# dbdexter-dev/meteor_demod

Measured on AMD Instinct MI355X. Metric: IQ Msamples/s demodulated (whole node), higher is better.
Workload: dtype f32

## Files before the change

meteor_demod_amd/_capi.py:

```python
from __future__ import annotations

import ctypes as C
from pathlib import Path

import numpy as np

LIB_DIR = Path(__file__).resolve().parent / "lib"
LIB_PATH = LIB_DIR / "libmeteor_demod_amd.so"
import os as _os
if _os.environ.get("MDEMOD_LIB_PATH"):
    LIB_PATH = Path(_os.environ["MDEMOD_LIB_PATH"])

MDEMOD_OK = 0
MDEMOD_ERR_PARAM = -1
MDEMOD_ERR_NOMEM = -2
MDEMOD_ERR_HIP = -3
MDEMOD_ERR_OVERFLOW = -4
MDEMOD_ERR_RANGE = -5
MDEMOD_MAX_LOCK_EVENTS = 32
MDEMOD_FLAG_KERNEL_MASK, MDEMOD_FLAG_LAT_OFF, MDEMOD_FLAG_LAT_ON, MDEMOD_FLAG_V2_PACKED, MDEMOD_FLAG_NO_CLOCK_JUMP = 0x3, 0x4, 0x8, 0x10, 0x20


def variant_flags_from_env() -> int:
    f = {"v1": 1, "v3": 3}.get(_os.environ.get("MDEMOD_KERNEL", ""), 0)
# ... 27 lines not shown
        ("locked", C.c_int32), ("locked_once", C.c_int32), ("overflow", C.c_int32),
    ]


class MdemodLockEvent(C.Structure):
    _fields_ = [("symbol", C.c_uint64), ("locked", C.c_int32), ("pad", C.c_int32)]


class MdemodStreamState(C.Structure):
    _fields_ = [
        ("agc_gain", C.c_float), ("agc_bias_re", C.c_float), ("agc_bias_im", C.c_float),
        ("pll_phase", C.c_float), ("pll_freq", C.c_float), ("pll_err", C.c_float),
        ("pll_locked", C.c_int32), ("pll_locked_once", C.c_int32), ("pll_updown", C.c_int32),
        ("t_phase", C.c_float), ("t_freq", C.c_float), ("t_prev", C.c_float),
        ("t_dual_state", C.c_int32), ("oqpsk_inphase", C.c_float),
        ("n_samples", C.c_uint64), ("n_symbols", C.c_uint64),
        ("first_lock_symbol", C.c_int64),
    ]


class MdemodRecordingOpts(C.Structure):
    _fields_ = [("tile_samples", C.c_uint32), ("acquire_samples", C.c_uint32), ("frame_samples", C.c_uint32),
                ("settle_samples", C.c_uint32), ("pilot_block", C.c_uint32), ("pilot_margin_symbols", C.c_uint32),
                ("max_pilot_samples", C.c_uint64), ("match_symbols", C.c_uint32), ("repair", C.c_int32),
                ("carrier_seed", C.c_uint32), ("clock_seed", C.c_uint32), ("debug", C.c_int32), ("debug_tile", C.c_int32)]


class MdemodRecordingReport(C.Structure):
    _fields_ = [("n_symbols", C.c_uint64), ("pilot_samples", C.c_uint64), ("pilot_symbols", C.c_uint64),
                ("exact_symbols", C.c_uint64), ("first_lock_symbol", C.c_int64), ("samples_demodulated", C.c_uint64),
                ("n_tiles", C.c_uint32), ("tile_samples", C.c_uint32), ("weak_seams", C.c_uint32), ("seam_fixes", C.c_uint32),
                ("pilot_locked", C.c_int32), ("weak_carrier_tiles", C.c_uint32),
                ("pilot_seconds", C.c_double), ("tiles_seconds", C.c_double),
                ("frame_misses", C.c_uint32), ("repaired_tiles", C.c_uint32), ("rotation_jumps", C.c_uint32),
                ("frame_residual_rms", C.c_float), ("odd_tiles_kept", C.c_uint32), ("weak_clock_tiles", C.c_uint32)]


_P = C.POINTER
SIGNATURES = {
    "mdemod_abi_version": (C.c_uint32, []),
    "mdemod_last_error": (C.c_char_p, []),
    "mdemod_strerror": (C.c_char_p, [C.c_int]),
    "mdemod_init_device": (C.c_int, [C.c_int]),
    "mdemod_create": (C.c_int, [_P(MdemodParams), _P(C.c_void_p)]),
    "mdemod_destroy": (None, [C.c_void_p]),
    "mdemod_reset": (C.c_int, [C.c_void_p, C.c_void_p]),
    "mdemod_max_symbols": (C.c_uint64, [C.c_void_p, C.c_uint64]),
    "mdemod_process_device_uniform": (C.c_int, [C.c_void_p, C.c_void_p, C.c_uint64, C.c_uint32,
                                                C.c_void_p, C.c_uint64, C.c_uint32, C.c_void_p]),
    "mdemod_process_device": (C.c_int, [C.c_void_p, C.c_void_p, C.c_void_p, C.c_void_p,
                                        C.c_void_p, C.c_uint64, C.c_uint32, C.c_void_p]),
    "mdemod_process_host": (C.c_int, [C.c_void_p, _P(C.c_void_p), _P(C.c_uint32),
                                      _P(C.c_void_p), _P(C.c_uint32), _P(C.c_uint32)]),
    "mdemod_pin_host_buffer": (C.c_int, [C.c_void_p, C.c_void_p, C.c_size_t]),
    "mdemod_unpin_host_buffer": (C.c_int, [C.c_void_p, C.c_void_p]),
    "mdemod_get_status": (C.c_int, [C.c_void_p, C.c_uint32, C.c_uint32, _P(MdemodStatus), C.c_void_p]),
    "mdemod_get_lock_events": (C.c_int, [C.c_void_p, C.c_uint32, _P(MdemodLockEvent), C.c_uint32,
                                         _P(C.c_uint32), C.c_void_p]),
    "mdemod_get_state": (C.c_int, [C.c_void_p, C.c_uint32, _P(MdemodStreamState), C.c_void_p]),
    "mdemod_set_state": (C.c_int, [C.c_void_p, C.c_uint32, _P(MdemodStreamState), C.c_void_p]),
    "mdemod_set_state_all": (C.c_int, [C.c_void_p, _P(MdemodStreamState), C.c_void_p]),
    "mdemod_rotate_carrier": (C.c_int, [C.c_void_p, C.c_void_p, C.c_void_p]),
    "mdemod_set_carrier_seeds": (C.c_int, [C.c_void_p, C.c_void_p, C.c_void_p, C.c_void_p]),
    "mdemod_set_gain_seeds": (C.c_int, [C.c_void_p, C.c_void_p, C.c_void_p]),
    "mdemod_set_clock_seeds": (C.c_int, [C.c_void_p, C.c_void_p, C.c_void_p]),
    "mdemod_get_states": (C.c_int, [C.c_void_p, C.c_uint32, C.c_uint32, _P(MdemodStreamState), C.c_void_p]),
    "mdemod_copy_state": (C.c_int, [C.c_void_p, C.c_void_p, C.c_void_p]),
    "mdemod_nominal_pitch": (C.c_uint64, [C.c_void_p, C.c_uint64]),
    "mdemod_compact_soft": (C.c_int, [C.c_void_p, C.c_void_p, C.c_uint64, C.c_void_p, C.c_uint64, C.c_void_p]),
    "mdemod_fanin_peer": (C.c_int, [C.c_void_p, C.c_void_p, C.c_uint64, C.c_int, C.c_void_p, C.c_uint64, C.c_uint64, C.c_void_p, C.c_void_p]),
    "mdemod_carrier_window_samples": (C.c_uint32, [C.c_void_p, C.c_uint32]),
    "mdemod_estimate_carrier": (C.c_int, [C.c_void_p, C.c_void_p, C.c_uint64, C.c_void_p, C.c_uint32, C.c_uint32,
                                          C.c_void_p, C.c_void_p, C.c_void_p]),
    "mdemod_estimate_carrier_chirp": (C.c_int, [C.c_void_p, C.c_void_p, C.c_uint64, C.c_void_p, C.c_void_p, C.c_uint32, C.c_uint32,
                                                C.c_void_p, C.c_void_p, C.c_void_p]),
    "mdemod_estimate_clock": (C.c_int, [C.c_void_p, C.c_void_p, C.c_uint64, C.c_void_p, C.c_void_p, C.c_void_p, C.c_uint32, C.c_uint32,
                                        C.c_void_p, C.c_void_p, C.c_void_p]),
    "mdemod_kernel_name": (C.c_char_p, [C.c_void_p]),
    "mdemod_plan_kernel": (C.c_int, [C.c_void_p, C.c_char_p, C.c_uint32, C.POINTER(C.c_uint32), C.POINTER(C.c_uint32)]),
    "mdemod_clock_interp_magic": (C.c_uint32, [C.c_int32]),
    "mdemod_clock_table": (C.c_int, [C.c_int32, C.c_int32, _P(C.c_int32), C.c_uint32]),
    "mdemod_plan_clock_table": (C.c_int, [C.c_void_p, _P(C.c_int32), C.c_uint32]),
    "mdemod_plan_launch": (C.c_int, [C.c_void_p, _P(C.c_int32)]),
    "mdemod_device_count": (C.c_int, []),
    "mdemod_demodulate_recording_host": (C.c_int, [_P(MdemodParams), _P(MdemodRecordingOpts), C.c_void_p, C.c_uint64,
                                                   C.c_void_p, C.c_uint64, _P(MdemodRecordingReport)]),
    "mdemod_recording_default_opts": (None, [_P(MdemodRecordingOpts)]),
    "mdemod_demodulate_recording": (C.c_int, [_P(MdemodParams), _P(MdemodRecordingOpts), C.c_void_p, C.c_uint64,
                                              C.c_void_p, C.c_uint64, _P(MdemodRecordingReport), C.c_void_p]),
    "mdemod_history_len": (C.c_uint32, [C.c_void_p]),
    "mdemod_get_history": (C.c_int, [C.c_void_p, C.c_uint32, _P(C.c_float), C.c_void_p]),
    "mdemod_set_history": (C.c_int, [C.c_void_p, C.c_uint32, _P(C.c_float), C.c_void_p]),
    "mdemod_derive_tables": (C.c_int, [_P(MdemodParams), _P(C.c_float), C.c_uint32,
                                       _P(C.c_float), _P(C.c_float)]),
    "mdemod_get_rrc_table": (C.c_int, [C.c_void_p, _P(C.c_float), C.c_uint32]),
    "mdemod_get_loop_constants": (C.c_int, [C.c_void_p, _P(C.c_float)]),
    "mdemod_get_tanh_lut": (C.c_int, [C.c_void_p, _P(C.c_float)]),
    "mdemod_selftest_sincos": (C.c_int, [C.c_void_p, _P(C.c_float), C.c_uint32, _P(C.c_float), _P(C.c_float)]),
    "mdemod_selftest_hypot": (C.c_int, [C.c_void_p, _P(C.c_float), C.c_uint32, _P(C.c_float)]),
    "mdemod_selftest_turncode": (C.c_int, [C.c_void_p, _P(C.c_uint64), _P(C.c_uint64)]),
    "mdemod_selftest_sinlut": (C.c_int, [C.c_void_p, _P(C.c_uint64), _P(C.c_uint64)]),
    "mdemod_selftest_cabsf": (C.c_int, [C.c_void_p, C.c_uint64, _P(C.c_uint64), _P(C.c_uint64)]),
    "mdemod_selftest_seam_match": (C.c_int, [C.c_int, C.c_void_p, C.c_uint64, C.c_void_p, C.c_uint64, C.c_void_p, C.c_void_p, C.c_void_p,
                                             C.c_void_p, C.c_void_p, C.c_void_p, C.c_uint32, C.c_int, C.c_void_p, C.c_void_p, C.c_void_p, C.c_void_p]),
    "mdemod_selftest_assemble": (C.c_int, [C.c_void_p, C.c_uint64, C.c_void_p, C.c_uint64, C.c_void_p, C.c_void_p, C.c_void_p, C.c_void_p,
                                           C.c_void_p, C.c_void_p, C.c_uint32, C.c_void_p]),
    "mdemod_selftest_window_power": (C.c_int, [C.c_void_p, C.c_void_p, C.c_uint64, C.c_void_p, C.c_void_p, C.c_uint32, C.c_void_p, C.c_void_p]),
}

_lib = None


class MdemodError(RuntimeError):
    def __init__(self, code: int, what: str):
        self.code = code
        self.detail = last_error()
        super().__init__(f"{what}: error {code} ({strerror(code)})" + (f": {self.detail}" if self.detail else ""))


def hip_runtime_first() -> None:
    try:
        import torch
    except ImportError:
        pass


def lib() -> C.CDLL:
    global _lib
    if _lib is None:
        hip_runtime_first()
        if not LIB_PATH.exists():
            raise RuntimeError(
                f"{LIB_PATH} is missing: build the HIP extension first "
                "(python -m meteor_demod_amd.build). There is no CPU fallback.")
        _lib = _typed(C.CDLL(str(LIB_PATH)), SIGNATURES, missing_ok=bool(_os.environ.get("MDEMOD_LIB_PATH")))
    return _lib


def _typed(handle: C.CDLL, *tables: dict, missing_ok: bool = False) -> C.CDLL:
    for table in tables:
        for name, (res, args) in table.items():
            if missing_ok and not hasattr(handle, name):
                continue
            fn = getattr(handle, name)
            fn.restype = res
            fn.argtypes = args
    return handle


def bind(*tables: dict) -> C.CDLL:
    return _typed(lib(), *tables)


def take_bytes(ptr, count: int, dtype=np.uint8) -> np.ndarray:
    dtype = np.dtype(dtype)
    return np.frombuffer(C.string_at(ptr, count * dtype.itemsize), dtype=dtype).copy() if count else np.zeros(0, dtype=dtype)


def strerror(code: int) -> str:
    return lib().mdemod_strerror(code).decode()


def last_error() -> str:
    fn = getattr(lib(), "mdemod_last_error", None)
    return (fn() or b"").decode(errors="replace") if fn is not None else ""

# ... 6 lines not shown
```

meteor_demod_amd/csrc/demod_api.cpp:

```cpp
#include <hip/hip_runtime.h>

#include <cmath>
#include <cstdio>
#include <cstdlib>
#include <cstring>
#include <new>
#include <vector>

#include "demod_host.h"
#include "demod_internal.h"
#include "hip_host.h"

struct mdemod_ctx {
	mdemod_params params;
	HostTables    tab;
	int           block_threads;
	size_t        lds_bytes;
	size_t        sample_bytes;

	DemodStateSoA st;
	float        *d_ctab;
	float        *d_lut;
	int32_t      *d_clock_tab;
	float        *d_rrc;
	int           hyb_block;
	bool          v1_global_table;
	bool          use_rot;
	bool          lat_ok;
	int           lat_ring, lat_span;
	size_t        lat_lds;
	MdmDevMem     mem;

	void   *pipe;
};

namespace {

template <typename T>
int
fetch(const T *dev, uint32_t first, uint32_t count, std::vector<T> &host, hipStream_t st)
{
	host.resize(count);
	HIP_TRY(hipMemcpyAsync(host.data(), dev + first, sizeof(T) * count, hipMemcpyDeviceToHost, st));
	return MDEMOD_OK;
}

bool
wants_latency_kernel(const mdemod_ctx *ctx)
{
	if (!ctx->lat_ok || (ctx->params.reserved & MDEMOD_FLAG_LAT_OFF)) return false;
	if (ctx->params.reserved & MDEMOD_FLAG_LAT_ON) return true;
	const double per_firing = static_cast<double>(ctx->tab.osf) / (ctx->params.oqpsk ? 2.0 : 1.0);
	if (ctx->tab.use_rw && per_firing > 32.0) return false;
	const uint32_t most = (ctx->tab.use_rw && (ctx->tab.rw_mid || ctx->tab.rw_far)) ? 1024u : (per_firing >= 8.0 ? 2048u : 4096u);
	return ctx->params.n_streams <= most;
}

struct LaunchPick {
	int kind;
	int geom;
	int many_slides;
	int compact;
	int long_filter;
};

LaunchPick
pick_launch(const mdemod_ctx *ctx)
{
	LaunchPick p = { MDEMOD_LAUNCH_V1, 0, 0, 0, 0 };
	const int geom = ctx->tab.rw_mid ? 1 : (ctx->tab.rw_far ? 2 : 0);
	if (wants_latency_kernel(ctx)) p.kind = MDEMOD_LAUNCH_LAT;
	else if (ctx->tab.use_rw && ctx->tab.rw_gather) { p.kind = MDEMOD_LAUNCH_GAT; p.long_filter = ctx->tab.c.taps > 65 ? 1 : 0; }
	else if (ctx->tab.use_rw && ctx->tab.rw_hyb) {
		p.kind = MDEMOD_LAUNCH_ROTH; p.geom = geom;
		p.many_slides = static_cast<double>(ctx->tab.osf) / (ctx->params.oqpsk ? 2.0 : 1.0) > 20.0 ? 1 : 0;
	}
	else if (ctx->tab.use_rw && ctx->use_rot) { p.kind = MDEMOD_LAUNCH_ROT; p.compact = ctx->tab.rw_std_compact ? 1 : 0; }
	else if (ctx->tab.use_rw && ctx->tab.rw_compact4) { p.kind = MDEMOD_LAUNCH_ROTP; p.geom = geom; }
	else if (ctx->tab.use_rw) p.kind = -1;
	return p;
}

int
launch(mdemod_ctx *ctx, DemodLaunch &L, hipStream_t stream)
{
	L.c = ctx->tab.c;
	L.st = ctx->st;
	L.n_streams = ctx->params.n_streams;
	L.ctab = ctx->d_ctab;
	L.ctab_floats = static_cast<uint32_t>(ctx->tab.ctab.size());
	L.tanh_lut = ctx->d_lut;
	L.c.clock_tab = ctx->d_clock_tab;
	const LaunchPick p = pick_launch(ctx);
	switch (p.kind) {
// ... 597 lines not shown
mdemod_fanin_peer(mdemod_ctx *src, const int8_t *soft_dev, uint64_t soft_stride_symbols, int dst_device,
                  int8_t *dst_soft_dev, uint64_t pitch_symbols, uint64_t first_row, uint32_t *dst_counts_dev, void *hip_stream)
try { MDEMOD_API_ENTER
	if (!src || !soft_dev || !dst_soft_dev || (soft_stride_symbols & 7) || (pitch_symbols & 7) || dst_device < 0) return MDEMOD_ERR_PARAM;
	int rc = mdm_select_device(src->params.device);
	if (rc) return rc;
	const int src_device = src->params.device;
	if (dst_device != src_device) {
		int can = 0;
		HIP_TRY(hipDeviceCanAccessPeer(&can, src_device, dst_device));
		if (!can) {
			mdm_note_error("mdemod_fanin_peer: device %d cannot reach the memory of device %d (no peer access between them)", src_device, dst_device);
			return MDEMOD_ERR_HIP;
		}
		const hipError_t e = hipDeviceEnablePeerAccess(dst_device, 0);
		if (e == hipErrorPeerAccessAlreadyEnabled) (void)hipGetLastError();
		else HIP_TRY(e);
	}
	hipStream_t st = static_cast<hipStream_t>(hip_stream);
	const uint32_t n = src->params.n_streams;
	HIP_TRY(mdemod_launch_compact_rows(soft_dev, soft_stride_symbols, dst_soft_dev + 2 * first_row * pitch_symbols, pitch_symbols,
	                                   src->st.sym_this_call, n, st));
	if (dst_counts_dev)
		HIP_TRY(hipMemcpyPeerAsync(dst_counts_dev + first_row, dst_device, src->st.sym_this_call, src_device, sizeof(uint32_t) * n, st));
	return MDEMOD_OK;
} MDEMOD_API_CATCH

const char *
mdemod_kernel_name(const mdemod_ctx *ctx)
{
	if (!ctx) return "";
	if (wants_latency_kernel(ctx)) return "demod_kernel_lat (one stream per wave: FIR farm + serial scalar stage)";
	if (!ctx->tab.use_rw) return "demod_kernel (v1 LDS ring)";
	if (ctx->tab.rw_gather) return ctx->tab.c.taps > 65 ? "demod_kernel_gat (v3 gather: sample rates beyond every window, 129 taps, every firing loads its own taps)"
	                                                     : "demod_kernel_gat (v3 gather: sample rates beyond every window, 65 taps, every firing loads its own taps)";
	if (ctx->tab.rw_hyb && ctx->tab.rw_far) return "demod_kernel_roth (v3 hybrid window, far: float input, 65 taps at up to 54 samples per firing, 80 slots in VGPRs + 40 in AccVGPRs)";
	if (ctx->tab.rw_hyb) return ctx->tab.rw_mid ? "demod_kernel_roth (v3 hybrid window, mid: float input, 65 taps at up to 30 samples per firing, 80 slots in VGPRs + 16 in AccVGPRs)"
	                                            : "demod_kernel_roth (v3 hybrid window: float input, 129 taps, 80 slots in VGPRs + 80 in AccVGPRs)";
	if (ctx->tab.rw_compact4) return ctx->tab.rw_wide ? "demod_kernel_rotp (v3 rotating packed window, wide: 129 taps at up to 30 samples per firing)"
	                                 : (ctx->tab.rw_mid ? "demod_kernel_rotp (v3 rotating packed window, mid: 65 taps at up to 15 samples per firing)"
	                                                    : "demod_kernel_rotp (v3 rotating packed window, far: 65 taps at up to 46 samples per firing)");
	return "demod_kernel_rot (v3 rotating register window)";
}

int
mdemod_plan_kernel(const mdemod_params *params, char *name, uint32_t name_cap, uint32_t *lds_bytes, uint32_t *block_threads)
try { MDEMOD_API_ENTER
	if (!params || !name || name_cap == 0 || params->n_streams == 0) return MDEMOD_ERR_PARAM;
	mdemod_ctx *ctx = new (std::nothrow) mdemod_ctx();
	if (!ctx) return MDEMOD_ERR_NOMEM;
	ctx->params = *params;
	ctx->pipe = nullptr;
	const int rc = plan_context(ctx);
	if (rc == MDEMOD_OK) {
		snprintf(name, name_cap, "%s%s", mdemod_kernel_name(ctx), ctx->v1_global_table && !wants_latency_kernel(ctx) ? " [table in global memory]" : "");
		if (lds_bytes) *lds_bytes = static_cast<uint32_t>(wants_latency_kernel(ctx) ? ctx->lat_lds : ctx->lds_bytes);
		if (block_threads) *block_threads = wants_latency_kernel(ctx) ? 64u : static_cast<uint32_t>(ctx->tab.use_rw ? (ctx->tab.rw_wide ? MDEMOD_RW_WIDE_BLOCK : (ctx->tab.c.sin_lut ? MDEMOD_RW_LUT_BLOCK : MDEMOD_RW_BLOCK)) : ctx->block_threads);
	}
	delete ctx;
	return rc;
} MDEMOD_API_CATCH

int
mdemod_plan_clock_table(const mdemod_params *params, int32_t *out, uint32_t cap_entries)
try { MDEMOD_API_ENTER
	if (!params || params->n_streams == 0) return MDEMOD_ERR_PARAM;
	mdemod_ctx *ctx = new (std::nothrow) mdemod_ctx();
	if (!ctx) return MDEMOD_ERR_NOMEM;
	ctx->params = *params;
	ctx->pipe = nullptr;
	int rc = plan_context(ctx);
	if (rc == MDEMOD_OK) {
		const size_t entries = ctx->tab.clock_tab.size() / 4;
		if (out && entries > cap_entries) rc = MDEMOD_ERR_PARAM;
		else {
			if (out && entries) memcpy(out, ctx->tab.clock_tab.data(), ctx->tab.clock_tab.size() * sizeof(int32_t));
			rc = static_cast<int>(entries);
		}
	}
	delete ctx;
	return rc;
} MDEMOD_API_CATCH

int
mdemod_plan_launch(const mdemod_params *params, int32_t out[MDEMOD_PLAN_LAUNCH_WORDS])
try { MDEMOD_API_ENTER
	if (!params || !out || params->n_streams == 0) return MDEMOD_ERR_PARAM;
	mdemod_ctx *ctx = new (std::nothrow) mdemod_ctx();
	if (!ctx) return MDEMOD_ERR_NOMEM;
	ctx->params = *params;
	ctx->pipe = nullptr;
	int rc = plan_context(ctx);
	if (rc == MDEMOD_OK) {
		const LaunchPick p = pick_launch(ctx);
		const DemodConsts &c = ctx->tab.c;
		const bool lat = p.kind == MDEMOD_LAUNCH_LAT, v1 = p.kind == MDEMOD_LAUNCH_V1;
		const int32_t v[MDEMOD_PLAN_LAUNCH_WORDS] = {
			p.kind, params->bps, c.oqpsk ? 1 : 0, c.step_safe, c.sin_lut ? 1 : 0, ctx->tab.clock_tab.empty() ? 0 : 1,
			p.geom, p.many_slides, p.compact, p.long_filter,
			v1 ? ctx->block_threads : 0, v1 && ctx->v1_global_table ? 1 : 0, v1 ? c.win_granules : 0,
			lat && ctx->tab.use_rw ? 1 : 0, 0, 0 };
		memcpy(out, v, sizeof(v));
		if (p.kind < 0) rc = MDEMOD_ERR_PARAM;
	}
	delete ctx;
	return rc;
} MDEMOD_API_CATCH

uint32_t
mdemod_history_len(const mdemod_ctx *ctx)
{
	return ctx ? static_cast<uint32_t>(ctx->tab.c.hpad) : 0;
}

int
mdemod_get_history(mdemod_ctx *ctx, uint32_t stream, float *iq_pairs, void *hip_stream)
try { MDEMOD_API_ENTER
	if (!ctx || !iq_pairs) return MDEMOD_ERR_PARAM;
	if (stream >= ctx->params.n_streams) return MDEMOD_ERR_RANGE;
	int rc = mdm_select_device(ctx->params.device);
	if (rc) return rc;
	hipStream_t st = static_cast<hipStream_t>(hip_stream);
	const int hfmt = ctx->tab.use_rw ? 32 : ctx->params.bps;
	const size_t sb = 2 * static_cast<size_t>(hfmt) / 8, ns = ctx->params.n_streams;
	const int hpad = ctx->tab.c.hpad;
	std::vector<unsigned char> raw(static_cast<size_t>(hpad) * sb);
	if (ctx->tab.use_rw)
		HIP_TRY(hipMemcpyAsync(raw.data(), static_cast<const unsigned char *>(ctx->st.hist) + static_cast<size_t>(stream) * hpad * sb,
		                       static_cast<size_t>(hpad) * sb, hipMemcpyDeviceToHost, st));
	else
		HIP_TRY(hipMemcpy2DAsync(raw.data(), sb, static_cast<const unsigned char *>(ctx->st.hist) + stream * sb,
		                         ns * sb, sb, hpad, hipMemcpyDeviceToHost, st));
	HIP_TRY(hipStreamSynchronize(st));
	for (int k = 0; k < hpad; k++) {
		const unsigned char *p = &raw[k * sb];
		if (hfmt == 8) { iq_pairs[2*k] = (float)((int)p[0] - 128); iq_pairs[2*k+1] = (float)((int)p[1] - 128); }
		else if (hfmt == 16) { int16_t v[2]; memcpy(v, p, 4); iq_pairs[2*k] = v[0]; iq_pairs[2*k+1] = v[1]; }
		else memcpy(&iq_pairs[2*k], p, 8);
	}
	return MDEMOD_OK;
} MDEMOD_API_CATCH

int
mdemod_set_history(mdemod_ctx *ctx, uint32_t stream, const float *iq_pairs, void *hip_stream)
try { MDEMOD_API_ENTER
	if (!ctx || !iq_pairs) return MDEMOD_ERR_PARAM;
	if (stream >= ctx->params.n_streams) return MDEMOD_ERR_RANGE;
	int rc = mdm_select_device(ctx->params.device);
	if (rc) return rc;
	hipStream_t st = static_cast<hipStream_t>(hip_stream);
	const int hfmt = ctx->tab.use_rw ? 32 : ctx->params.bps;
	const size_t sb = 2 * static_cast<size_t>(hfmt) / 8, ns = ctx->params.n_streams;
	const int hpad = ctx->tab.c.hpad;
	std::vector<unsigned char> raw(static_cast<size_t>(hpad) * sb);
	for (int k = 0; k < hpad; k++) {
		unsigned char *p = &raw[k * sb];
		const float re = iq_pairs[2*k], im = iq_pairs[2*k+1];
		if (hfmt == 8) {
			if (re != floorf(re) || im != floorf(im) || re < -128 || re > 127 || im < -128 || im > 127) return MDEMOD_ERR_PARAM;
			p[0] = (unsigned char)((int)re + 128); p[1] = (unsigned char)((int)im + 128);
		} else if (hfmt == 16) {
			if (re != floorf(re) || im != floorf(im) || re < -32768 || re > 32767 || im < -32768 || im > 32767) return MDEMOD_ERR_PARAM;
			int16_t v[2] = { (int16_t)re, (int16_t)im }; memcpy(p, v, 4);
		} else memcpy(p, &iq_pairs[2*k], 8);
	}
	if (ctx->tab.use_rw)
// ... 107 lines not shown
```

meteor_demod_amd/csrc/demod_kernel_gat.hip:

```cpp
#include "rotwin_body.h"
#include "hip_host.h"

namespace {

typedef float gpair_t __attribute__((ext_vector_type(2)));
typedef float gquad_t __attribute__((ext_vector_type(4)));
typedef __attribute__((address_space(3))) const gquad_t lds_gquad;
typedef __attribute__((address_space(3))) const float lds_gfloat;

template <int FMT> struct GFmt;
template <> struct GFmt<16> {
	enum { G = 4 };
	__device__ static __forceinline__ gpair_t get(const uint4 &q, int k) { const uint32_t w = (&q.x)[k]; return gpair_t{ (float)(int)(int16_t)(w & 0xFFFFu), (float)((int)w >> 16) }; }
	__device__ static __forceinline__ gpair_t one(uint32_t w) { return gpair_t{ (float)(int)(int16_t)(w & 0xFFFFu), (float)((int)w >> 16) }; }
};
template <> struct GFmt<8> {
	enum { G = 8 };
	__device__ static __forceinline__ gpair_t get(const uint4 &q, int k) { const uint32_t w = (&q.x)[k >> 1] >> (16 * (k & 1)); return gpair_t{ (float)((int)(w & 0xFFu) - 128), (float)((int)((w >> 8) & 0xFFu) - 128) }; }
	__device__ static __forceinline__ gpair_t one(uint16_t w) { return gpair_t{ (float)((int)(w & 0xFFu) - 128), (float)((int)(w >> 8) - 128) }; }
};
template <> struct GFmt<32> {
	enum { G = 2 };
	__device__ static __forceinline__ gpair_t get(const uint4 &q, int k) { return gpair_t{ __uint_as_float((&q.x)[2 * k]), __uint_as_float((&q.x)[2 * k + 1]) }; }
	__device__ static __forceinline__ gpair_t one(float2 w) { return gpair_t{ w.x, w.y }; }
};

template <int KT, int FMT>
struct WinG {
	static constexpr int G = GFmt<FMT>::G, kTaps = KT, kBack = KT - 1, AMAX = G - 1, NS = KT + AMAX, NW = 4 * ((NS + 3) / 4), SLIDE = 4, MAXSL = 1, DEPTH = 1,
	                     BLOCK = MDEMOD_RW_BLOCK, ROTN = 1, RING = 32, REGSLOTS = 0;
	static constexpr bool GATHER = true, SCALAR_SLIDE = false, VCONST = false;
	static_assert(NS % G == 0 && NS / G <= 36, "whole 16-byte loads, and few enough of them to stay in registers");
	typedef typename RFmt<FMT>::sample_t sample_t;
	__device__ __forceinline__ void setup(uint32_t) {}
	__device__ static __forceinline__ void put_history(const float2 *, bool, int) {}
	__device__ static __forceinline__ void put_init(const RGran<FMT> (&)[1], int) {}
	__device__ static __forceinline__ void put(const RGran<FMT> (&)[1], int) {}
	__device__ static __forceinline__ void fir(uint32_t, int, int, const DemodConsts &, int, float &, float &) {}

	__device__ static __forceinline__ void
	fir_gather(uint32_t ctab_addr, const sample_t *src, const float2 *hist, int v, int n, int bank, const DemodConsts &C, float &re, float &im)
	{
		const int oldest = v - kBack - (KT - 1);
		const int d = oldest & (G - 1);
		const int start = oldest - d;
		const int o = AMAX - d;
		const uint32_t row = ctab_addr + 4u * (uint32_t)(__mul24(bank * 4 + (o & 3), C.ctab_row_stride) + (o & ~3));
		gpair_t acc = { 0.0f, 0.0f };
		if (__builtin_expect(md_all(start >= 0 && start + NS <= n), 1)) {
			uint4 raw[NS / G];
#pragma unroll
			for (int g = 0; g < NS / G; g++) __builtin_memcpy(&raw[g], src + start + G * g, 16);
#pragma unroll
			for (int s4 = 0; s4 < NS / 4; s4++) {
				gquad_t c = { 0.0f, 0.0f, 0.0f, 0.0f };
				c = *(lds_gquad *)(row + 16u * (uint32_t)s4);
				const float cf[4] = { c.x, c.y, c.z, c.w };
#pragma unroll
				for (int k = 0; k < 4; k++) {
					const int slot = 4 * s4 + k;
					const gpair_t smp = GFmt<FMT>::get(raw[slot / G], slot % G);
					const gpair_t p = smp * cf[k];
					acc = acc + p;
				}
			}
			if constexpr (NS % 4 != 0) {
#pragma unroll
				for (int slot = NS / 4 * 4; slot < NS; slot++) {
					const float cf = *(lds_gfloat *)(row + 4u * (uint32_t)slot);
					const gpair_t p = GFmt<FMT>::get(raw[slot / G], slot % G) * cf;
					acc = acc + p;
				}
			}
		} else {
#pragma unroll 1
			for (int k = 0; k < KT; k++) {
				const int idx = oldest + k;
				gpair_t smp;
				if (idx < 0) { const float2 h = hist[kBack + idx]; smp.x = h.x; smp.y = h.y; }
				else smp = GFmt<FMT>::one(src[idx]);
				const float cf = *(lds_gfloat *)(row + 4u * (uint32_t)(d + k));
				const gpair_t p = smp * cf;
				acc = acc + p;
			}
		}
		re = acc.x; im = acc.y;
	}
};

template <int FMT, int OQPSK, int KT>
__global__ void __launch_bounds__(MDEMOD_RW_BLOCK, 2)
demod_kernel_gat(const DemodLaunch L)
{
	rotwin_demod<WinG<KT, FMT>, FMT, OQPSK, 0>(L);
}

template <int FMT, int OQPSK, int KT>
hipError_t
launch_gat(const DemodLaunch &L, size_t lds_bytes, hipStream_t stream)
{
	const uint32_t blocks = (L.n_streams + MDEMOD_RW_BLOCK - 1) / MDEMOD_RW_BLOCK;
	auto kfn = demod_kernel_gat<FMT, OQPSK, KT>;
	return mdm_launch(kfn, dim3(blocks), dim3(MDEMOD_RW_BLOCK), lds_bytes, stream, L);
}

}

template <int FMT>
static hipError_t
launch_gat_fmt(const DemodLaunch &L, int long_filter, size_t lds_bytes, hipStream_t stream)
{
	if constexpr (FMT != 32)
		if (long_filter) return L.c.oqpsk ? launch_gat<FMT, 1, 129>(L, lds_bytes, stream) : launch_gat<FMT, 0, 129>(L, lds_bytes, stream);
// ... 15 lines not shown
```

meteor_demod_amd/csrc/demod_kernel_rot.hip:

```cpp
#include "rotwin_body.h"
#include "rot_fir_bounds.h"
#include "hip_host.h"
#ifdef ROTWIN_ASM_HEADER
#include ROTWIN_ASM_HEADER
#else
#include "rotwin_asm.h"
#endif

namespace {

static_assert(ROTWIN_NCH * 8 == 80 && ROTWIN_SLIDE == 8, "window = ten chunks of eight, a slide brings one");


__device__ __forceinline__ void
rot_fir(uint32_t row_addr, int rot, int flags, float &re, float &im)
{
	int tmp;
#if ROTWIN_PK == 1 || ROTWIN_PK == 3
	typedef float pair_t __attribute__((ext_vector_type(2)));
	pair_t acc, p0, p1;
	asm volatile(ROTWIN_FIR_ASM
	             : [acc] "=&v"(acc), [p0] "=&v"(p0), [p1] "=&v"(p1), [tmp] "=&s"(tmp)
	             : [addr] "v"(row_addr), [rot] "s"(rot), [flags] "s"(flags)
	             : "vcc", "scc", ROTWIN_COEF_CLOBBERS);
	re = acc.x; im = acc.y;
#else
	float t0, t1, t2, t3;
	asm volatile(ROTWIN_FIR_ASM
	             : [ar] "=&v"(re), [ai] "=&v"(im), [t0] "=&v"(t0), [t1] "=&v"(t1), [t2] "=&v"(t2), [t3] "=&v"(t3), [tmp] "=&s"(tmp)
	             : [addr] "v"(row_addr), [rot] "s"(rot), [flags] "s"(flags)
	             : "vcc", "scc", ROTWIN_COEF_CLOBBERS);
#endif
}

template <int FMT> __device__ __forceinline__ void rot_put(const RGran<FMT> &a, const RGran<FMT> &b, int &q, int &base);
template <> __device__ __forceinline__ void
rot_put<16>(const RGran<16> &a, const RGran<16> &b, int &q, int &base)
{
	int tmp;
	asm volatile(ROTWIN_PUT_S16_ASM
	             : [tmp] "=&s"(tmp), [rot] "+s"(q), [base] "+s"(base)
	             : [g0] "v"(a.w[0]), [g1] "v"(a.w[1]), [g2] "v"(a.w[2]), [g3] "v"(a.w[3]),
	               [g4] "v"(b.w[0]), [g5] "v"(b.w[1]), [g6] "v"(b.w[2]), [g7] "v"(b.w[3])
	             : "vcc", "scc", "v255", "memory");
}
template <> __device__ __forceinline__ void
rot_put<8>(const RGran<8> &a, const RGran<8> &b, int &q, int &base)
{
	const uint32_t g0 = a.w[0] ^ 0x80808080u, g1 = a.w[1] ^ 0x80808080u, g2 = b.w[0] ^ 0x80808080u, g3 = b.w[1] ^ 0x80808080u;
	int tmp;
	asm volatile(ROTWIN_PUT_U8_ASM
	             : [tmp] "=&s"(tmp), [rot] "+s"(q), [base] "+s"(base)
	             : [g0] "v"(g0), [g1] "v"(g1), [g2] "v"(g2), [g3] "v"(g3)
	             : "vcc", "scc", "v255", "memory");
}
__device__ __forceinline__ void
rot_put_floats(const uint32_t (&f)[16], int &q, int &base)
{
	int tmp;
	asm volatile(ROTWIN_PUT_F32_ASM
	             : [tmp] "=&s"(tmp), [rot] "+s"(q), [base] "+s"(base)
	             : [f0] "v"(f[0]), [f1] "v"(f[1]), [f2] "v"(f[2]), [f3] "v"(f[3]), [f4] "v"(f[4]), [f5] "v"(f[5]), [f6] "v"(f[6]), [f7] "v"(f[7]),
	               [f8] "v"(f[8]), [f9] "v"(f[9]), [f10] "v"(f[10]), [f11] "v"(f[11]), [f12] "v"(f[12]), [f13] "v"(f[13]), [f14] "v"(f[14]), [f15] "v"(f[15])
	             : "vcc", "scc", "v255", "memory");
}
__device__ __forceinline__ void
rot_put_floats(const uint32_t (&f)[16], int q)
{
	int base = 0;
	rot_put_floats(f, q, base);
}
template <> __device__ __forceinline__ void
rot_put<32>(const RGran<32> &a, const RGran<32> &b, int &q, int &base)
{
	uint32_t f[16];
#pragma unroll
	for (int i = 0; i < 8; i++) { f[i] = a.w[i]; f[8 + i] = b.w[i]; }
	rot_put_floats(f, q, base);
}

template <int FMT, int COMPACT = 0, int BLK = MDEMOD_RW_BLOCK, int VC = 0, int RSL = 0>
struct WinF {
	static constexpr int kTaps = 65, kBack = 64, NW = 80, SLIDE = 8, AMAX = NW - kTaps, MAXSL = 1, DEPTH = 1, BLOCK = BLK, ROTN = NW / SLIDE, RING = 32;
	static constexpr bool GATHER = false;
	static constexpr bool SCALAR_SLIDE = true;
	static constexpr bool VCONST = VC != 0;
	static_assert(SLIDE == ROTWIN_SLIDE && ROTN == ROTWIN_NCH, "the slide's assembly counts for itself");
	__device__ __forceinline__ void setup(uint32_t) {}
	static constexpr int REGSLOTS = RSL;
	__device__ static __forceinline__ void put_history(const float2 *hist, bool valid, int q)
	{
		const uint4 *h4 = reinterpret_cast<const uint4 *>(hist);
		uint32_t f[16];
#pragma unroll
		for (int i = 0; i < 4; i++) {
			uint4 h = h4[i];
			if (!valid) h = make_uint4(0, 0, 0, 0);
			f[4 * i] = h.x; f[4 * i + 1] = h.y; f[4 * i + 2] = h.z; f[4 * i + 3] = h.w;
		}
		rot_put_floats(f, q);
	}
	__device__ static __forceinline__ void put(const RGran<FMT> (&g)[2], int q) { int base = 0; rot_put<FMT>(g[0], g[1], q, base); }
	__device__ static __forceinline__ void put_init(const RGran<FMT> (&g)[2], int q) { put(g, q); }
	__device__ static __forceinline__ void slide(const RGran<FMT> (&g)[2], int &rot, int &base) { rot_put<FMT>(g[0], g[1], rot, base); }
	__device__ static __forceinline__ void fir(uint32_t ctab_addr, int a, int bank, const DemodConsts &C, int rot, float &re, float &im)
	{
		const int o = AMAX - a;
		uint32_t row_addr;
		if (COMPACT) row_addr = rot_mad24((uint32_t)(bank * 4 + (o & 3)), 4u * (uint32_t)C.ctab_row_stride, ctab_addr + 4u * (uint32_t)(o & ~3));
		else row_addr = rot_mad24(rot_mad24((uint32_t)a, (uint32_t)C.interp, (uint32_t)bank), 4u * (uint32_t)C.ctab_row_stride, ctab_addr);
		static_assert(AMAX == 15, "two bits of a / 4");
		const uint64_t ex = __builtin_amdgcn_ballot_w64(true);
		const RotFirQ q = rot_fir_q(ex, __builtin_amdgcn_ballot_w64(a >= 4), __builtin_amdgcn_ballot_w64(a >= 8), __builtin_amdgcn_ballot_w64(a >= 12));
		int q_hi = q.q_hi;
		asm("" : "+s"(q_hi));
		const int flags = rot_fir_flags(q.q_lo, q_hi);
#ifdef ROT_EXP_NOSKIP
		int f0 = __builtin_amdgcn_readfirstlane(flags);
		asm volatile("s_and_b32 %0, %0, 0" : "+s"(f0) : : "scc");
		rot_fir(row_addr, rot, f0, re, im);
#else
		rot_fir(row_addr, rot, flags, re, im);
#endif
	}
};

typedef float pair_t2 __attribute__((ext_vector_type(2)));

template <int NA>
__device__ __forceinline__ void
rot_fir_acc(uint32_t addr, int rot, int last, pair_t2 &acc)
{
	int tmp;
	if constexpr (NA == 10)
		asm volatile(ROTWIN_FIR_ACC_ASM
		             : [acc] "+v"(acc), [tmp] "=&s"(tmp)
		             : [addr] "v"(addr), [rot] "s"(rot), [last] "s"(last)
		             : "vcc", "scc", ROTWIN_COEF_CLOBBERS, ROTWIN_ACC_CLOBBERS);
	else if constexpr (NA == 2)
		asm volatile(ROTWIN_FIR_ACC2_ASM
		             : [acc] "+v"(acc), [tmp] "=&s"(tmp)
		             : [addr] "v"(addr), [rot] "s"(rot), [last] "s"(last)
		             : "vcc", "scc", ROTWIN_COEF_CLOBBERS, ROTWIN_ACC_CLOBBERS);
	else
		asm volatile(ROTWIN_FIR_ACC5_ASM
		             : [acc] "+v"(acc), [tmp] "=&s"(tmp)
		             : [addr] "v"(addr), [rot] "s"(rot), [last] "s"(last)
		             : "vcc", "scc", ROTWIN_COEF_CLOBBERS, ROTWIN_ACC_CLOBBERS);
}
#define ROT_F16_OPERANDS \
	[f0] "v"(f[0]), [f1] "v"(f[1]), [f2] "v"(f[2]), [f3] "v"(f[3]), [f4] "v"(f[4]), [f5] "v"(f[5]), [f6] "v"(f[6]), [f7] "v"(f[7]), \
	[f8] "v"(f[8]), [f9] "v"(f[9]), [f10] "v"(f[10]), [f11] "v"(f[11]), [f12] "v"(f[12]), [f13] "v"(f[13]), [f14] "v"(f[14]), [f15] "v"(f[15])
template <int NA>
__device__ __forceinline__ void
rot_migrate(const uint32_t (&f)[16], int q)
{
	int tmp;
	if constexpr (NA == 10)
		asm volatile(ROTWIN_MIGRATE_ASM : [tmp] "=&s"(tmp) : ROT_F16_OPERANDS, [rot] "s"(q) : "vcc", "scc", "v255", ROTWIN_ACC_CLOBBERS, "memory");
	else if constexpr (NA == 2)
		asm volatile(ROTWIN_MIGRATE2_ASM : [tmp] "=&s"(tmp) : ROT_F16_OPERANDS, [rot] "s"(q) : "vcc", "scc", "v255", ROTWIN_ACC_CLOBBERS, "memory");
	else
		asm volatile(ROTWIN_MIGRATE5_ASM : [tmp] "=&s"(tmp) : ROT_F16_OPERANDS, [rot] "s"(q) : "vcc", "scc", "v255", ROTWIN_ACC_CLOBBERS, "memory");
}
template <int NA>
__device__ __forceinline__ void
rot_put_acc(const uint32_t (&f)[16], int q)
{
	int tmp;
	if constexpr (NA == 10)
		asm volatile(ROTWIN_PUT_ACC_ASM : [tmp] "=&s"(tmp) : ROT_F16_OPERANDS, [rot] "s"(q) : "vcc", "scc", ROTWIN_ACC_CLOBBERS, "memory");
	else if constexpr (NA == 2)
		asm volatile(ROTWIN_PUT_ACC2_ASM : [tmp] "=&s"(tmp) : ROT_F16_OPERANDS, [rot] "s"(q) : "vcc", "scc", ROTWIN_ACC_CLOBBERS, "memory");
	else
		asm volatile(ROTWIN_PUT_ACC5_ASM : [tmp] "=&s"(tmp) : ROT_F16_OPERANDS, [rot] "s"(q) : "vcc", "scc", ROTWIN_ACC_CLOBBERS, "memory");
}

template <int BLK, int NA, int MSL>
struct WinH {
	static constexpr int NR = 10, SLIDE = 8, NW = SLIDE * (NR + NA), kTaps = NA == 10 ? 129 : 65, kBack = kTaps - 1, AMAX = NW - kTaps, MAXSL = MSL, DEPTH = MSL,
	                     BLOCK = BLK, ROTN = NR, RING = 32, REGSLOTS = 0;
	static constexpr bool GATHER = false, SCALAR_SLIDE = false, VCONST = false;
	static_assert((NA == 10 || NA == 2 || NA == 5) && AMAX == (NA == 5 ? 55 : 31) && kBack % SLIDE == 0, "wide (160 slots, 129 taps), mid (96 slots, 65 taps) or far (120 slots, 65 taps)");
	__device__ __forceinline__ void setup(uint32_t) {}
	__device__ static __forceinline__ void place(const uint32_t (&f)[16], int c)
	{
		if (c < NR) rot_put_floats(f, c);
		else rot_put_acc<NA>(f, c - NR);
	}
	__device__ static __forceinline__ void put_history(const float2 *hist, bool valid, int c)
	{
		const uint4 *h4 = reinterpret_cast<const uint4 *>(hist);
		uint32_t f[16];
#pragma unroll
		for (int i = 0; i < 4; i++) {
			uint4 h = h4[i];
			if (!valid) h = make_uint4(0, 0, 0, 0);
			f[4 * i] = h.x; f[4 * i + 1] = h.y; f[4 * i + 2] = h.z; f[4 * i + 3] = h.w;
		}
		place(f, c);
	}
	__device__ static __forceinline__ void put_init(const RGran<32> (&g)[2], int c)
	{
		uint32_t f[16];
#pragma unroll
		for (int i = 0; i < 8; i++) { f[i] = g[0].w[i]; f[8 + i] = g[1].w[i]; }
		place(f, c);
	}
	__device__ static __forceinline__ void put(const RGran<32> (&g)[2], int q)
	{
		uint32_t f[16];
#pragma unroll
		for (int i = 0; i < 8; i++) { f[i] = g[0].w[i]; f[8 + i] = g[1].w[i]; }
		rot_migrate<NA>(f, q);
	}
	__device__ static __forceinline__ void fir(uint32_t ctab_addr, int a, int bank, const DemodConsts &C, int rot, float &re, float &im)
	{
		const int o = AMAX - a;
		const uint32_t row = ctab_addr + 4u * (uint32_t)(__mul24(bank * 4 + (o & 3), C.ctab_row_stride) + (o & ~3));
		const int flags = (md_all(a >= 8) ? 3 : 0) | ((NA != 10 && md_all(a <= 7)) ? 16 : 0);
		rot_fir(row, rot, __builtin_amdgcn_readfirstlane(flags), re, im);
		if (NA == 10 || md_any(a >= 16)) {
			int last;
			if (NA == 10) last = 6 + (md_any(a >= 8) ? 1 : 0) + (md_any(a >= 16) ? 1 : 0) + (md_any(a >= 24) ? 1 : 0);
			else {
				last = md_any(a >= 24) ? 1 : 0;
				if (NA == 5) last += (md_any(a >= 32) ? 1 : 0) + (md_any(a >= 40) ? 1 : 0) + (md_any(a >= 48) ? 1 : 0);
			}
			pair_t2 acc = { re, im };
			rot_fir_acc<NA>(row + 4u * 80u, NA == 10 ? rot : (NA == 2 ? (rot & 1) : (rot >= 5 ? rot - 5 : rot)), __builtin_amdgcn_readfirstlane(last), acc);
			re = acc.x; im = acc.y;
		}
	}
};

template <int OQPSK, int BLK, int NA, int MSL>
__global__ void __launch_bounds__(BLK, 1) __attribute__((amdgpu_num_vgpr(ROTWIN_LIMIT)))
demod_kernel_roth(const DemodLaunch L)
{
	rotwin_demod<WinH<BLK, NA, MSL>, 32, OQPSK, 0>(L);
}

#ifndef ROT_VCONST
#define ROT_VCONST 1
#endif
template <int FMT, int OQPSK, int KS, int COMPACT, int LUT>
constexpr int rot_regslots() { return 15; }
template <int FMT, int OQPSK, int KS, int COMPACT, int LUT>
__global__ void __launch_bounds__(LUT ? MDEMOD_RW_LUT_BLOCK : MDEMOD_RW_BLOCK, 2) __attribute__((amdgpu_num_vgpr(ROTWIN_LIMIT / 2)))
demod_kernel_rot(const DemodLaunch L)
{
	rotwin_demod<WinF<FMT, COMPACT, LUT ? MDEMOD_RW_LUT_BLOCK : MDEMOD_RW_BLOCK, ROT_VCONST, rot_regslots<FMT, OQPSK, KS, COMPACT, LUT>()>, FMT, OQPSK, KS, LUT>(L);
}

template <int FMT, int OQPSK, int KS, int COMPACT = 0, int LUT = 0>
hipError_t
launch_rot_ks(const DemodLaunch &L, size_t lds_bytes, hipStream_t stream)
{
	constexpr int BLOCK = LUT ? MDEMOD_RW_LUT_BLOCK : MDEMOD_RW_BLOCK;
	const uint32_t blocks = (L.n_streams + BLOCK - 1) / BLOCK;
	auto kfn = demod_kernel_rot<FMT, OQPSK, KS, COMPACT, LUT>;
	return mdm_launch(kfn, dim3(blocks), dim3(BLOCK), lds_bytes, stream, L);
}

template <int FMT, int OQPSK>
hipError_t
launch_rot(const DemodLaunch &L, int compact, size_t lds_bytes, hipStream_t stream)
{
	constexpr int KS = OQPSK ? 6 : 14;
	if (compact) return launch_rot_ks<FMT, OQPSK, 0, 1>(L, lds_bytes, stream);
	return L.c.sin_lut && L.c.step_safe == KS && L.c.clock_tab ? launch_rot_ks<FMT, OQPSK, KS, 0, 1>(L, lds_bytes, stream) : launch_rot_ks<FMT, OQPSK, 0>(L, lds_bytes, stream);
}

}

template <int OQPSK, int BLK, int NA, int MSL>
static hipError_t
launch_roth(const DemodLaunch &L, size_t lds_bytes, hipStream_t stream)
{
	const uint32_t blocks = (L.n_streams + BLK - 1) / BLK;
	auto kfn = demod_kernel_roth<OQPSK, BLK, NA, MSL>;
	return mdm_launch(kfn, dim3(blocks), dim3(BLK), lds_bytes, stream, L);
}

hipError_t
mdemod_launch_demod_roth(const DemodLaunch &L, int geom, int many_slides, size_t lds_bytes, hipStream_t stream)
{
	if (geom == 1 && many_slides) return L.c.oqpsk ? launch_roth<1, 256, 2, 3>(L, lds_bytes, stream) : launch_roth<0, 256, 2, 3>(L, lds_bytes, stream);
	if (geom == 1) return L.c.oqpsk ? launch_roth<1, 256, 2, 2>(L, lds_bytes, stream) : launch_roth<0, 256, 2, 2>(L, lds_bytes, stream);
	if (geom == 2) return L.c.oqpsk ? launch_roth<1, 256, 5, 3>(L, lds_bytes, stream) : launch_roth<0, 256, 5, 3>(L, lds_bytes, stream);
	return L.c.oqpsk ? launch_roth<1, 256, 10, 2>(L, lds_bytes, stream) : launch_roth<0, 256, 10, 2>(L, lds_bytes, stream);
}

hipError_t
mdemod_launch_demod_rot(const DemodLaunch &L, int fmt, int compact, size_t lds_bytes, hipStream_t stream)
{
	switch (fmt) {
	case 16: return L.c.oqpsk ? launch_rot<16, 1>(L, compact, lds_bytes, stream) : launch_rot<16, 0>(L, compact, lds_bytes, stream);
	case 8:  return L.c.oqpsk ? launch_rot<8, 1>(L, compact, lds_bytes, stream) : launch_rot<8, 0>(L, compact, lds_bytes, stream);
	case 32: return L.c.oqpsk ? launch_rot<32, 1>(L, compact, lds_bytes, stream) : launch_rot<32, 0>(L, compact, lds_bytes, stream);
	default: return hipErrorInvalidValue;
	}
}
```

meteor_demod_amd/csrc/demod_kernel_rotp.hip:

```cpp
#include "rotwin_body.h"
#include "hip_host.h"
#ifdef ROTPK_ASM_HEADER
#include ROTPK_ASM_HEADER
#else
#include "rotpk_asm.h"
#endif

namespace {

typedef float pair_t __attribute__((ext_vector_type(2)));

template <int GEO> struct GeoP;
#ifndef ROTP_WIDE_DEPTH
#define ROTP_WIDE_DEPTH 1
#endif
#ifndef ROTP_MID_DEPTH
#define ROTP_MID_DEPTH 1
#endif
#ifndef ROTP_FAR_DEPTH
#define ROTP_FAR_DEPTH 2
#endif
template <> struct GeoP<0> { static constexpr int kTaps = 129, NW = MDEMOD_RW_WIDE_NW, MAXSL = 1, DEPTH = ROTP_WIDE_DEPTH, BLOCK = MDEMOD_RW_WIDE_BLOCK; };
template <> struct GeoP<1> { static constexpr int kTaps = 65, NW = MDEMOD_RW_MID_NW, MAXSL = 1, DEPTH = ROTP_MID_DEPTH, BLOCK = MDEMOD_RW_BLOCK; };
#ifndef ROTP_FAR_MAXSL
#define ROTP_FAR_MAXSL 2
#endif
template <> struct GeoP<2> { static constexpr int kTaps = 65, NW = MDEMOD_RW_FAR_NW, MAXSL = ROTP_FAR_MAXSL, DEPTH = ROTP_FAR_DEPTH, BLOCK = MDEMOD_RW_BLOCK; };
static_assert(MDEMOD_RW_WIDE_NW == 160 && MDEMOD_RW_MID_NW == 96 && MDEMOD_RW_FAR_NW == 112, "gen_rotpk_asm.py: GEOS");

template <int GEO, int FMT> struct AsmP;
#if ROTPK_FORM == 0
#define ROTP_FIR_CALL(TEXT, CLOB)                                                                                             \
	float ar = 0.0f, ai = 0.0f;                                                                                               \
	asm volatile(TEXT : [ar] "+v"(ar), [ai] "+v"(ai), [addr] "+v"(addr), [cnt] "+s"(cnt), [tmp] "=&s"(tmp)                    \
	             : [entry] "s"(entry), [sub] "s"(sub) : "vcc", "scc", CLOB);                                                \
	re = ar; im = ai;
#else
#define ROTP_FIR_CALL(TEXT, CLOB)                                                                                             \
	pair_t acc = { 0.0f, 0.0f };                                                                                              \
	asm volatile(TEXT : [acc] "+v"(acc), [addr] "+v"(addr), [cnt] "+s"(cnt), [tmp] "=&s"(tmp)                                 \
	             : [entry] "s"(entry), [sub] "s"(sub) : "vcc", "scc", CLOB);                                                \
	re = acc.x; im = acc.y;
#endif
#define ROTP_ASM(GEO, NAME, FMT)                                                                                              \
	template <> struct AsmP<GEO, FMT> {                                                                                       \
		__device__ static __forceinline__ void fir(uint32_t addr, int entry, int sub, int cnt, float &re, float &im)          \
		{                                                                                                                     \
			int tmp;                                                                                                          \
			ROTP_FIR_CALL(ROTPK_##NAME##_##FMT##_FIR_ASM, ROTPK_##NAME##_##FMT##_CLOBBERS)                                     \
		}                                                                                                                     \
		__device__ static __forceinline__ void put(const uint32_t (&g)[FMT == 16 ? 16 : 8], int q);                           \
	};
ROTP_ASM(0, WIDE, 16) ROTP_ASM(0, WIDE, 8) ROTP_ASM(1, MID, 16) ROTP_ASM(1, MID, 8) ROTP_ASM(2, FAR, 16) ROTP_ASM(2, FAR, 8)

#define ROTP_PUT16(GEO, NAME)                                                                                                 \
	__device__ __forceinline__ void AsmP<GEO, 16>::put(const uint32_t (&g)[16], int q)                                        \
	{                                                                                                                         \
		int tmp;                                                                                                              \
		asm volatile(ROTPK_##NAME##_16_PUT_ASM                                                                                \
		             : [tmp] "=&s"(tmp)                                                                                       \
		             : [g0] "v"(g[0]), [g1] "v"(g[1]), [g2] "v"(g[2]), [g3] "v"(g[3]), [g4] "v"(g[4]), [g5] "v"(g[5]), [g6] "v"(g[6]),  \
		               [g7] "v"(g[7]), [g8] "v"(g[8]), [g9] "v"(g[9]), [g10] "v"(g[10]), [g11] "v"(g[11]), [g12] "v"(g[12]),  \
		               [g13] "v"(g[13]), [g14] "v"(g[14]), [g15] "v"(g[15]), [rot] "s"(q)                                     \
		             : "vcc", "scc", "v255", "memory");                                                                       \
	}
#define ROTP_PUT8(GEO, NAME)                                                                                                  \
	__device__ __forceinline__ void AsmP<GEO, 8>::put(const uint32_t (&g)[8], int q)                                          \
	{                                                                                                                         \
		int tmp;                                                                                                              \
		asm volatile(ROTPK_##NAME##_8_PUT_ASM                                                                                 \
		             : [tmp] "=&s"(tmp)                                                                                       \
		             : [g0] "v"(g[0]), [g1] "v"(g[1]), [g2] "v"(g[2]), [g3] "v"(g[3]), [g4] "v"(g[4]), [g5] "v"(g[5]), [g6] "v"(g[6]),  \
		               [g7] "v"(g[7]), [rot] "s"(q)                                                                           \
		             : "vcc", "scc", "v255", "memory");                                                                       \
	}
ROTP_PUT16(0, WIDE) ROTP_PUT16(1, MID) ROTP_PUT16(2, FAR) ROTP_PUT8(0, WIDE) ROTP_PUT8(1, MID) ROTP_PUT8(2, FAR)

template <int GEO, int FMT>
struct WinP {
	static constexpr int kTaps = GeoP<GEO>::kTaps, kBack = kTaps - 1, NW = GeoP<GEO>::NW, SLIDE = 16, AMAX = NW - kTaps,
	                     MAXSL = GeoP<GEO>::MAXSL, DEPTH = GeoP<GEO>::DEPTH, BLOCK = GeoP<GEO>::BLOCK, NCH = NW / SLIDE, GD = FMT == 16 ? 16 : 8, REGSLOTS = 0, ROTN = NCH, RING = 32;
	static constexpr bool GATHER = false, SCALAR_SLIDE = false, VCONST = false;
	__device__ __forceinline__ void setup(uint32_t) {}
	static_assert(kBack % SLIDE == 0 && NW % SLIDE == 0, "history and window are whole chunks");

	__device__ static __forceinline__ void put_history(const float2 *hist, bool valid, int q)
	{
		uint32_t g[GD];
#pragma unroll
		for (int k = 0; k < 16; k++) {
			float2 h = hist[k];
			if (!valid) h = make_float2(0.0f, 0.0f);
			if (FMT == 16) {
				g[k] = ((uint32_t)(int)h.x & 0xFFFFu) | ((uint32_t)(int)h.y << 16);
			} else {
				const uint32_t s = (uint32_t)(((int)h.x + 128) & 0xFF) | ((uint32_t)(((int)h.y + 128) & 0xFF) << 8);
				if (k & 1) g[k / 2] |= s << 16; else g[k / 2] = s;
			}
		}
		AsmP<GEO, FMT>::put(g, q);
	}
	__device__ static __forceinline__ void put(const RGran<FMT> (&gr)[4], int q)
	{
		uint32_t g[GD];
#pragma unroll
		for (int i = 0; i < 4; i++)
#pragma unroll
			for (int j = 0; j < GD / 4; j++) g[i * (GD / 4) + j] = gr[i].w[j];
		AsmP<GEO, FMT>::put(g, q);
	}
	__device__ static __forceinline__ void put_init(const RGran<FMT> (&gr)[4], int q) { put(gr, q); }
	__device__ static __forceinline__ void fir(uint32_t ctab_addr, int a, int bank, const DemodConsts &C, int rot, float &re, float &im)
	{
		const int o = AMAX - a;
		uint32_t addr = rot_mad24((uint32_t)(bank * 4 + (o & 3)), 4u * (uint32_t)C.ctab_row_stride, ctab_addr + 4u * (uint32_t)(o & ~3));
		constexpr int QB = AMAX / 4 >= 8 ? 4 : 3;
		static_assert(AMAX / 4 < (1 << QB) && (kTaps - 1) % 4 == 0, "alignments in groups of four");
		int q_lo = 0, q_hi = (1 << QB) - 1;
#pragma unroll
		for (int b = QB - 1; b >= 0; b--) {
			const int t = q_lo + (1 << b);
			q_lo = md_all(a >= 4 * t) ? t : q_lo;
			const int u = q_hi - (1 << b);
			q_hi = md_all(a < 4 * (u + 1)) ? u : q_hi;
		}
		q_lo = __builtin_amdgcn_readfirstlane(q_lo); q_hi = __builtin_amdgcn_readfirstlane(q_hi);
		const int c_lo = q_lo >> 2;
		int chunk = rot + c_lo;
		chunk = chunk >= NCH ? chunk - NCH : chunk;
		const int sub = q_lo & 3;
		constexpr int XS = ROTPK_EXIT / 4;
		const int cnt = (q_hi + (kTaps - 1) / 4) / XS - q_lo / XS;
		AsmP<GEO, FMT>::fir(addr + 64u * (uint32_t)c_lo, __builtin_amdgcn_readfirstlane(chunk), __builtin_amdgcn_readfirstlane(sub), __builtin_amdgcn_readfirstlane(cnt), re, im);
	}
};

#define ROTP_KERNEL(GEO, NAME, FMT, OQ)                                                                                       \
	__global__ void __launch_bounds__(GeoP<GEO>::BLOCK, 2) __attribute__((amdgpu_num_vgpr(ROTPK_##NAME##_##FMT##_LIMIT / 2)))  \
	demod_kernel_rotp_##NAME##_##FMT##_##OQ(const DemodLaunch L) { rotwin_demod<WinP<GEO, FMT>, FMT, OQ, 0>(L); }
__global__ void __launch_bounds__(GeoP<0>::BLOCK, 2) __attribute__((amdgpu_num_vgpr(ROTPK_WIDE_16_LIMIT / 2)))
demod_kernel_rotp_WIDE_16_0_ks109(const DemodLaunch L) { rotwin_demod<WinP<0, 16>, 16, 0, 109, 1>(L); }
ROTP_KERNEL(0, WIDE, 16, 0) ROTP_KERNEL(0, WIDE, 16, 1) ROTP_KERNEL(0, WIDE, 8, 0) ROTP_KERNEL(0, WIDE, 8, 1)
ROTP_KERNEL(1, MID, 16, 0) ROTP_KERNEL(1, MID, 16, 1) ROTP_KERNEL(1, MID, 8, 0) ROTP_KERNEL(1, MID, 8, 1)
ROTP_KERNEL(2, FAR, 16, 0) ROTP_KERNEL(2, FAR, 16, 1) ROTP_KERNEL(2, FAR, 8, 0) ROTP_KERNEL(2, FAR, 8, 1)

typedef void (*rotp_kernel_t)(const DemodLaunch);

hipError_t
launch_rotp(rotp_kernel_t kfn, int block, const DemodLaunch &L, size_t lds_bytes, hipStream_t stream)
{
	const uint32_t blocks = (L.n_streams + block - 1) / block;
	return mdm_launch(kfn, dim3(blocks), dim3(block), lds_bytes, stream, L);
}

}

hipError_t
mdemod_launch_demod_rotp(const DemodLaunch &L, int fmt, int geom , size_t lds_bytes, hipStream_t stream)
{
	if ((fmt != 16 && fmt != 8) || geom < 0 || geom > 2) return hipErrorInvalidValue;
	static const rotp_kernel_t table[3][2][2] = {
		{ { demod_kernel_rotp_WIDE_16_0, demod_kernel_rotp_WIDE_16_1 }, { demod_kernel_rotp_WIDE_8_0, demod_kernel_rotp_WIDE_8_1 } },
		{ { demod_kernel_rotp_MID_16_0, demod_kernel_rotp_MID_16_1 }, { demod_kernel_rotp_MID_8_0, demod_kernel_rotp_MID_8_1 } },
		{ { demod_kernel_rotp_FAR_16_0, demod_kernel_rotp_FAR_16_1 }, { demod_kernel_rotp_FAR_8_0, demod_kernel_rotp_FAR_8_1 } },
// ... 6 lines not shown
```

meteor_demod_amd/csrc/gen_rotwin_asm.py:

```python
#!/usr/bin/env python3
import os
import sys

WB = 96
CB = None
NCH = 10
SLIDE = 8
PAIRWAIT = int(os.environ.get("ROTWIN_PAIRWAIT", "1"))
DC = int(os.environ.get("ROTWIN_DC", "1"))
NBUF = 2 * (DC + 1) if PAIRWAIT else 4
CB = 96 - 4 * NBUF
PK = int(os.environ.get("ROTWIN_PK", "1"))
TB = CB - 4
CHB = 32


def q(lines):
    return "\n".join('\t"%s\\n\\t"' % l for l in lines)


def jump(tag, n):
    return [
        "s_getpc_b64 vcc",
        ".L%s_pc_%%=:" % tag,
# ... 14 lines not shown
    if PK in (0, 2):
        L += ["v_mov_b32 %[ar], 0", "v_mov_b32 %[ai], 0"]
    else:
        L += ["v_mov_b64 %[acc], 0"]
    L += [load(h) for h in range(2 * DC if PAIRWAIT else D)]
    L += jump("fir", NCH)
    for r in range(NCH):
        L += [".Lfir_%d_%%=:" % r]
        for h in range(NH):
            c = h // 2
            if PAIRWAIT:
                if h % 2 == 0:
                    L += [load(x) for x in (h + 2 * DC, h + 2 * DC + 1) if x < NH]
                    L += ["s_waitcnt lgkmcnt(%d)" % min(2 * DC, max(0, NH - 2 - h))]
            else:
                if h + D < NH:
                    L += [load(h + D)]
                L += ["s_waitcnt lgkmcnt(%d)" % min(D, NH - 1 - h)]
            if h < 3:
                L += ["s_bitcmp1_b32 %%[flags], %d" % h, "s_cbranch_scc1 .Lfir_%d_s%d_%%=" % (r, h)]
            if h >= NH - 3:
                L += ["s_bitcmp1_b32 %%[flags], %d" % (3 + NH - 1 - h), "s_cbranch_scc1 .Lfir_%d_s9_%%=" % r]
            hb = CB + 4 * (h % NBUF)
            wq = WB + 16 * ((c + r) % NCH) + 8 * (h & 1)
            if PK == 1:
                def mul(j):
                    return ["v_pk_mul_f32 %%[p%d], v[%d:%d], v[%d:%d] op_sel:[0,%d] op_sel_hi:[1,%d]"
                            % (j & 1, wq + 2 * j, wq + 2 * j + 1, hb + 2 * (j // 2), hb + 2 * (j // 2) + 1, j & 1, j & 1)]
                def add(j):
                    return ["v_pk_add_f32 %%[acc], %%[acc], %%[p%d]" % (j & 1)]
            elif PK == 2:
                def mul(j):
                    t = TB + 2 * (j & 1)
                    return ["v_pk_mul_f32 v[%d:%d], v[%d:%d], v[%d:%d] op_sel:[0,%d] op_sel_hi:[1,%d]"
                            % (t, t + 1, wq + 2 * j, wq + 2 * j + 1, hb + 2 * (j // 2), hb + 2 * (j // 2) + 1, j & 1, j & 1)]
                def add(j):
                    t = TB + 2 * (j & 1)
                    return ["v_add_f32 %%[ar], %%[ar], v%d" % t, "v_add_f32 %%[ai], %%[ai], v%d" % (t + 1)]
            elif PK == 3:
                def mul(j):
                    t = TB + 2 * (j & 1)
                    return ["v_mul_f32 v%d, v%d, v%d" % (t, hb + j, wq + 2 * j), "v_mul_f32 v%d, v%d, v%d" % (t + 1, hb + j, wq + 2 * j + 1)]
                def add(j):
                    t = TB + 2 * (j & 1)
                    return ["v_pk_add_f32 %%[acc], %%[acc], v[%d:%d]" % (t, t + 1)]
            else:
                def mul(j):
                    t = "%%[t%d]" % (2 * (j & 1)), "%%[t%d]" % (2 * (j & 1) + 1)
                    return ["v_mul_f32 %s, v%d, v%d" % (t[0], hb + j, wq + 2 * j),
                            "v_mul_f32 %s, v%d, v%d" % (t[1], hb + j, wq + 2 * j + 1)]
                def add(j):
                    t = "%%[t%d]" % (2 * (j & 1)), "%%[t%d]" % (2 * (j & 1) + 1)
                    return ["v_add_f32 %%[ar], %%[ar], %s" % t[0], "v_add_f32 %%[ai], %%[ai], %s" % t[1]]
            L += mul(0)
            for j in range(4):
                if j + 1 < 4:
                    L += mul(j + 1)
                L += add(j)
            if h < 3:
                L += [".Lfir_%d_s%d_%%=:" % (r, h)]
        L += [".Lfir_%d_s9_%%=:" % r, "s_branch .Lfir_end_%="]
    L += [".Lfir_end_%=:", "s_waitcnt lgkmcnt(0)"]
    return L


def put(kind):
    L = ["s_nop 1"] if kind == "u8" else []
    L += jump("put", NCH)
    for r in range(NCH):
        L += [".Lput_%d_%%=:" % r]
        wq = WB + 16 * r
        for s in range(8):
            for comp in range(2):
                dst = wq + 2 * s + comp
                if kind == "s16":
                    L += ["v_cvt_f32_i32_sdwa v%d, sext(%%[g%d]) dst_sel:DWORD dst_unused:UNUSED_PAD src0_sel:WORD_%d" % (dst, s, comp)]
                elif kind == "u8":
                    L += ["v_cvt_f32_i32_sdwa v%d, sext(%%[g%d]) dst_sel:DWORD dst_unused:UNUSED_PAD src0_sel:BYTE_%d" % (dst, s // 2, 2 * (s & 1) + comp)]
                else:
                    L += ["v_mov_b32 v%d, %%[f%d]" % (dst, 2 * s + comp)]
        L += ["s_branch .Lput_end_%="]
    L += [".Lput_end_%=:"]
    L += ["s_add_i32 %%[base], %%[base], %d" % SLIDE,
          "s_add_i32 %[rot], %[rot], 1",
          "s_cmp_eq_u32 %%[rot], %d" % NCH,
          "s_cselect_b32 %[rot], 0, %[rot]"]
    return L


AB = 96


def fir_acc(NA, tag):
    NH = 2 * NA
    lo = 6 if NA == NCH else 0
    def load(h):
        b = CB + 4 * (h % 3)
        return "ds_read_b128 v[%d:%d], %%[addr] offset:%d" % (b, b + 3, 16 * h)
    L = [load(h) for h in range(2)]
    L += jump(tag, NA)
    for r in range(NA):
        L += [".L%s_%d_%%=:" % (tag, r)]
        for h in range(NH):
            c = h // 2
            if h + 2 < NH:
                L += [load(h + 2)]
            L += ["s_waitcnt lgkmcnt(%d)" % min(2, NH - 1 - h)]
            hb = CB + 4 * (h % 3)
            aq = AB + 16 * ((c + r) % NA) + 8 * (h & 1)
            def rd(j):
                t = CB + 12 + 2 * (j & 1)
                return ["v_accvgpr_read_b32 v%d, a%d" % (t, aq + 2 * j), "v_accvgpr_read_b32 v%d, a%d" % (t + 1, aq + 2 * j + 1)]
            def mul(j):
                t = CB + 12 + 2 * (j & 1)
                return ["v_pk_mul_f32 v[%d:%d], v[%d:%d], v[%d:%d] op_sel:[0,%d] op_sel_hi:[1,%d]" % (t, t + 1, t, t + 1, hb + 2 * (j // 2), hb + 2 * (j // 2) + 1, j & 1, j & 1)]
            def add(j):
                t = CB + 12 + 2 * (j & 1)
                return ["v_pk_add_f32 %%[acc], %%[acc], v[%d:%d]" % (t, t + 1)]
            L += rd(0) + rd(1) + mul(0) + mul(1) + add(0) + rd(2) + add(1) + rd(3) + mul(2) + mul(3) + add(2) + add(3)
            if h % 2 == 1 and lo <= c < NA - 1:
                L += ["s_cmp_eq_u32 %%[last], %d" % c, "s_cbranch_scc1 .L%s_end_%%=" % tag]
        L += ["s_branch .L%s_end_%%=" % tag]
    L += [".L%s_end_%%=:" % tag, "s_waitcnt lgkmcnt(0)"]
    return L


def migrate(NA, tag):
    assert NCH % NA == 0
    L = jump(tag, NCH)
    for r in range(NCH):
        L += [".L%s_%d_%%=:" % (tag, r)]
        L += ["v_accvgpr_read_b32 v%d, a%d" % (WB + 16 * r + k, AB + 16 * (r % NA) + k) for k in range(16)]
        L += ["v_accvgpr_write_b32 a%d, %%[f%d]" % (AB + 16 * (r % NA) + k, k) for k in range(16)]
        L += ["s_branch .L%s_end_%%=" % tag]
    L += [".L%s_end_%%=:" % tag]
    return L


def put_acc(NA, tag):
    L = jump(tag, NA)
    for r in range(NA):
        L += [".L%s_%d_%%=:" % (tag, r)]
        L += ["v_accvgpr_write_b32 a%d, %%[f%d]" % (AB + 16 * r + k, k) for k in range(16)]
        L += ["s_branch .L%s_end_%%=" % tag]
    L += [".L%s_end_%%=:" % tag]
    return L


def main():
    out = []
    out.append("/* GENERATED by gen_rotwin_asm.py - do not edit.  gfx950 assembly of the rotating register window. */")
    out.append("#ifndef MDEMOD_ROTWIN_ASM_H")
    out.append("#define MDEMOD_ROTWIN_ASM_H")
    out.append("#define ROTWIN_WB %d" % WB)
    out.append("#define ROTWIN_CB %d" % CB)
    out.append("#define ROTWIN_LIMIT %d   /* first register the compiler may not use */" % (TB if PK in (2, 3) else CB))
    out.append("#define ROTWIN_NCH %d" % NCH)
    out.append("#define ROTWIN_SLIDE %d" % SLIDE)
    out.append("#define ROTWIN_AB %d   /* first AccVGPR of the hybrid window's newer half */" % AB)
    out.append("#define ROTWIN_PK %d" % PK)
    out.append("#define ROTWIN_FIR_ASM \\\n" + q(fir()).replace("\n", " \\\n"))
    for kind in ("s16", "u8", "f32"):
        out.append("#define ROTWIN_PUT_%s_ASM \\\n" % kind.upper() + q(put(kind)).replace("\n", " \\\n"))
    for NA, sfx in ((NCH, ""), (2, "2"), (5, "5")):
        out.append("#define ROTWIN_FIR_ACC%s_ASM \\\n" % sfx + q(fir_acc(NA, "fira" + sfx)).replace("\n", " \\\n"))
        out.append("#define ROTWIN_MIGRATE%s_ASM \\\n" % sfx + q(migrate(NA, "mig" + sfx)).replace("\n", " \\\n"))
# ... 10 lines not shown
```

meteor_demod_amd/csrc/mdemod_internal_api.h:

```cpp
#ifndef MDEMOD_INTERNAL_API_H
#define MDEMOD_INTERNAL_API_H

#include "../../include/meteor_demod_amd.h"

#ifdef __cplusplus
#include <new>
void mdm_note_error(const char *fmt, ...) __attribute__((format(printf, 1, 2)));
struct mdm_api_scope { mdm_api_scope(); ~mdm_api_scope(); };
#define MDEMOD_API_ENTER mdm_api_scope api_scope_;
#define MDEMOD_API_CATCH catch (...) { mdm_note_error("a C++ exception reached the boundary (allocation failed, or a thread could not be started)"); return MDEMOD_ERR_NOMEM; }
extern "C" {
#endif


int  mdemod_set_state_all(mdemod_ctx *ctx, const mdemod_stream_state *seed, void *hip_stream);
int  mdemod_rotate_carrier(mdemod_ctx *ctx, const int32_t *quarter_turns_dev, void *hip_stream);

int  mdemod_set_carrier_seeds(mdemod_ctx *ctx, const float *freq_dev, const int32_t *updown_dev, void *hip_stream);
int  mdemod_set_gain_seeds(mdemod_ctx *ctx, const float *gain_dev, void *hip_stream);

int  mdemod_set_clock_seeds(mdemod_ctx *ctx, const float *t_freq_dev, void *hip_stream);
int  mdemod_get_states(mdemod_ctx *ctx, uint32_t first, uint32_t count, mdemod_stream_state *out, void *hip_stream);
int  mdemod_copy_state(mdemod_ctx *dst, mdemod_ctx *src, void *hip_stream);

uint32_t mdemod_carrier_window_samples(const mdemod_params *params, uint32_t window_samples);
int  mdemod_estimate_carrier(const mdemod_params *params, const void *iq_dev, uint64_t n_samples,
                             const uint64_t *starts_dev, uint32_t n_windows, uint32_t window_samples,
                             float *freq_dev, float *quality_dev, void *hip_stream);
int  mdemod_estimate_carrier_chirp(const mdemod_params *params, const void *iq_dev, uint64_t n_samples,
                                   const uint64_t *starts_dev, const float *chirp_dev, uint32_t n_windows, uint32_t window_samples,
                                   float *freq_dev, float *quality_dev, void *hip_stream);
int  mdemod_estimate_clock(const mdemod_params *params, const void *iq_dev, uint64_t n_samples,
                           const uint64_t *starts_dev, const float *carrier_dev, const float *chirp_dev,
                           uint32_t n_windows, uint32_t window_samples, float *t_freq_dev, float *quality_dev, void *hip_stream);


int  mdemod_derive_tables(const mdemod_params *params, float *rrc_out, uint32_t rrc_cap,
                          float consts_out[8], float lut_out[32]);
int  mdemod_plan_kernel(const mdemod_params *params, char *name, uint32_t name_cap, uint32_t *lds_bytes, uint32_t *block_threads);

uint32_t mdemod_clock_interp_magic(int32_t interp);
int  mdemod_clock_table(int32_t interp, int32_t k_safe, int32_t *out, uint32_t cap_entries);
int  mdemod_plan_clock_table(const mdemod_params *params, int32_t *out, uint32_t cap_entries);

enum { MDEMOD_LAUNCH_LAT = 0, MDEMOD_LAUNCH_GAT = 1, MDEMOD_LAUNCH_ROTH = 2, MDEMOD_LAUNCH_ROT = 3, MDEMOD_LAUNCH_ROTP = 4, MDEMOD_LAUNCH_V1 = 5 };
#define MDEMOD_PLAN_LAUNCH_WORDS 16
int  mdemod_plan_launch(const mdemod_params *params, int32_t out[MDEMOD_PLAN_LAUNCH_WORDS]);

int  mdemod_get_rrc_table(const mdemod_ctx *ctx, float *out, uint32_t cap);
int  mdemod_get_loop_constants(const mdemod_ctx *ctx, float out[8]);
int  mdemod_get_tanh_lut(const mdemod_ctx *ctx, float out[32]);

int  mdemod_selftest_sincos(mdemod_ctx *ctx, const float *x, uint32_t n,
                            float *sin_out, float *cos_out);
int  mdemod_selftest_hypot(mdemod_ctx *ctx, const float *xy, uint32_t n_pairs, float *out);
int  mdemod_selftest_turncode(mdemod_ctx *ctx, uint64_t *n_checked, uint64_t *n_mismatch);
int  mdemod_selftest_cabsf(mdemod_ctx *ctx, uint64_t pairs, uint64_t *n_mismatch, uint64_t *n_fallback);
int  mdemod_selftest_sinlut(mdemod_ctx *ctx, uint64_t *n_checked, uint64_t *n_mismatch);



int  mdemod_selftest_seam_match(int mode, const int8_t *a_dev, uint64_t a_symbols, const int8_t *b_dev, uint64_t b_symbols,
                                const uint64_t *a_off, const uint32_t *a_cnt, const uint64_t *b_off, const uint32_t *b_cnt,
                                const int32_t *b_rot, const int32_t *force_weak, uint32_t n_pairs, int K,
                                int32_t *shift_out, int32_t *rot_out, int32_t *weak_out, void *hip_stream);
int  mdemod_selftest_assemble(const int8_t *src_dev, uint64_t src_symbols, int8_t *out_dev, uint64_t out_symbols,
                              const uint64_t *src_off, const uint32_t *keep, const int32_t *rot, const int64_t *head_off,
                              const int32_t *head_rot, const uint64_t *dst, uint32_t n_tiles, void *hip_stream);
int  mdemod_selftest_window_power(const mdemod_params *params, const void *iq_dev, uint64_t n_samples, const uint64_t *starts,
                                  const uint32_t *lens, uint32_t n_windows, float *power_out_host, void *hip_stream);

#ifdef __cplusplus
}
#endif
#endif
```

meteor_demod_amd/csrc/rotwin_asm.h:

```cpp
#ifndef MDEMOD_ROTWIN_ASM_H
#define MDEMOD_ROTWIN_ASM_H
#define ROTWIN_WB 96
#define ROTWIN_CB 80
#define ROTWIN_LIMIT 80
#define ROTWIN_NCH 10
#define ROTWIN_SLIDE 8
#define ROTWIN_AB 96
#define ROTWIN_PK 1
#define ROTWIN_FIR_ASM \
	"v_mov_b64 %[acc], 0\n\t" \
	"ds_read_b128 v[80:83], %[addr] offset:0\n\t" \
	"ds_read_b128 v[84:87], %[addr] offset:16\n\t" \
	"s_getpc_b64 vcc\n\t" \
	".Lfir_pc_%=:\n\t" \
	"s_mul_i32 %[tmp], %[rot], (.Lfir_1_%= - .Lfir_0_%=)\n\t" \
	"s_add_u32 %[tmp], %[tmp], (.Lfir_0_%= - .Lfir_pc_%=)\n\t" \
	"s_add_u32 vcc_lo, vcc_lo, %[tmp]\n\t" \
	"s_addc_u32 vcc_hi, vcc_hi, 0\n\t" \
	"s_setpc_b64 vcc\n\t" \
	".Lfir_0_%=:\n\t" \
	"ds_read_b128 v[88:91], %[addr] offset:32\n\t" \
	"ds_read_b128 v[92:95], %[addr] offset:48\n\t" \
	"s_waitcnt lgkmcnt(2)\n\t" \
	"s_bitcmp1_b32 %[flags], 0\n\t" \
// ... 2164 lines not shown
	"v_cvt_f32_i32_sdwa v184, sext(%[g4]) dst_sel:DWORD dst_unused:UNUSED_PAD src0_sel:WORD_0\n\t" \
	"v_cvt_f32_i32_sdwa v185, sext(%[g4]) dst_sel:DWORD dst_unused:UNUSED_PAD src0_sel:WORD_1\n\t" \
	"v_cvt_f32_i32_sdwa v186, sext(%[g5]) dst_sel:DWORD dst_unused:UNUSED_PAD src0_sel:WORD_0\n\t" \
	"v_cvt_f32_i32_sdwa v187, sext(%[g5]) dst_sel:DWORD dst_unused:UNUSED_PAD src0_sel:WORD_1\n\t" \
	"v_cvt_f32_i32_sdwa v188, sext(%[g6]) dst_sel:DWORD dst_unused:UNUSED_PAD src0_sel:WORD_0\n\t" \
	"v_cvt_f32_i32_sdwa v189, sext(%[g6]) dst_sel:DWORD dst_unused:UNUSED_PAD src0_sel:WORD_1\n\t" \
	"v_cvt_f32_i32_sdwa v190, sext(%[g7]) dst_sel:DWORD dst_unused:UNUSED_PAD src0_sel:WORD_0\n\t" \
	"v_cvt_f32_i32_sdwa v191, sext(%[g7]) dst_sel:DWORD dst_unused:UNUSED_PAD src0_sel:WORD_1\n\t" \
	"s_branch .Lput_end_%=\n\t" \
	".Lput_6_%=:\n\t" \
	"v_cvt_f32_i32_sdwa v192, sext(%[g0]) dst_sel:DWORD dst_unused:UNUSED_PAD src0_sel:WORD_0\n\t" \
	"v_cvt_f32_i32_sdwa v193, sext(%[g0]) dst_sel:DWORD dst_unused:UNUSED_PAD src0_sel:WORD_1\n\t" \
	"v_cvt_f32_i32_sdwa v194, sext(%[g1]) dst_sel:DWORD dst_unused:UNUSED_PAD src0_sel:WORD_0\n\t" \
	"v_cvt_f32_i32_sdwa v195, sext(%[g1]) dst_sel:DWORD dst_unused:UNUSED_PAD src0_sel:WORD_1\n\t" \
	"v_cvt_f32_i32_sdwa v196, sext(%[g2]) dst_sel:DWORD dst_unused:UNUSED_PAD src0_sel:WORD_0\n\t" \
	"v_cvt_f32_i32_sdwa v197, sext(%[g2]) dst_sel:DWORD dst_unused:UNUSED_PAD src0_sel:WORD_1\n\t" \
	"v_cvt_f32_i32_sdwa v198, sext(%[g3]) dst_sel:DWORD dst_unused:UNUSED_PAD src0_sel:WORD_0\n\t" \
	"v_cvt_f32_i32_sdwa v199, sext(%[g3]) dst_sel:DWORD dst_unused:UNUSED_PAD src0_sel:WORD_1\n\t" \
	"v_cvt_f32_i32_sdwa v200, sext(%[g4]) dst_sel:DWORD dst_unused:UNUSED_PAD src0_sel:WORD_0\n\t" \
	"v_cvt_f32_i32_sdwa v201, sext(%[g4]) dst_sel:DWORD dst_unused:UNUSED_PAD src0_sel:WORD_1\n\t" \
	"v_cvt_f32_i32_sdwa v202, sext(%[g5]) dst_sel:DWORD dst_unused:UNUSED_PAD src0_sel:WORD_0\n\t" \
	"v_cvt_f32_i32_sdwa v203, sext(%[g5]) dst_sel:DWORD dst_unused:UNUSED_PAD src0_sel:WORD_1\n\t" \
	"v_cvt_f32_i32_sdwa v204, sext(%[g6]) dst_sel:DWORD dst_unused:UNUSED_PAD src0_sel:WORD_0\n\t" \
	"v_cvt_f32_i32_sdwa v205, sext(%[g6]) dst_sel:DWORD dst_unused:UNUSED_PAD src0_sel:WORD_1\n\t" \
	"v_cvt_f32_i32_sdwa v206, sext(%[g7]) dst_sel:DWORD dst_unused:UNUSED_PAD src0_sel:WORD_0\n\t" \
	"v_cvt_f32_i32_sdwa v207, sext(%[g7]) dst_sel:DWORD dst_unused:UNUSED_PAD src0_sel:WORD_1\n\t" \
	"s_branch .Lput_end_%=\n\t" \
	".Lput_7_%=:\n\t" \
	"v_cvt_f32_i32_sdwa v208, sext(%[g0]) dst_sel:DWORD dst_unused:UNUSED_PAD src0_sel:WORD_0\n\t" \
	"v_cvt_f32_i32_sdwa v209, sext(%[g0]) dst_sel:DWORD dst_unused:UNUSED_PAD src0_sel:WORD_1\n\t" \
	"v_cvt_f32_i32_sdwa v210, sext(%[g1]) dst_sel:DWORD dst_unused:UNUSED_PAD src0_sel:WORD_0\n\t" \
	"v_cvt_f32_i32_sdwa v211, sext(%[g1]) dst_sel:DWORD dst_unused:UNUSED_PAD src0_sel:WORD_1\n\t" \
	"v_cvt_f32_i32_sdwa v212, sext(%[g2]) dst_sel:DWORD dst_unused:UNUSED_PAD src0_sel:WORD_0\n\t" \
	"v_cvt_f32_i32_sdwa v213, sext(%[g2]) dst_sel:DWORD dst_unused:UNUSED_PAD src0_sel:WORD_1\n\t" \
	"v_cvt_f32_i32_sdwa v214, sext(%[g3]) dst_sel:DWORD dst_unused:UNUSED_PAD src0_sel:WORD_0\n\t" \
	"v_cvt_f32_i32_sdwa v215, sext(%[g3]) dst_sel:DWORD dst_unused:UNUSED_PAD src0_sel:WORD_1\n\t" \
	"v_cvt_f32_i32_sdwa v216, sext(%[g4]) dst_sel:DWORD dst_unused:UNUSED_PAD src0_sel:WORD_0\n\t" \
	"v_cvt_f32_i32_sdwa v217, sext(%[g4]) dst_sel:DWORD dst_unused:UNUSED_PAD src0_sel:WORD_1\n\t" \
	"v_cvt_f32_i32_sdwa v218, sext(%[g5]) dst_sel:DWORD dst_unused:UNUSED_PAD src0_sel:WORD_0\n\t" \
	"v_cvt_f32_i32_sdwa v219, sext(%[g5]) dst_sel:DWORD dst_unused:UNUSED_PAD src0_sel:WORD_1\n\t" \
	"v_cvt_f32_i32_sdwa v220, sext(%[g6]) dst_sel:DWORD dst_unused:UNUSED_PAD src0_sel:WORD_0\n\t" \
	"v_cvt_f32_i32_sdwa v221, sext(%[g6]) dst_sel:DWORD dst_unused:UNUSED_PAD src0_sel:WORD_1\n\t" \
	"v_cvt_f32_i32_sdwa v222, sext(%[g7]) dst_sel:DWORD dst_unused:UNUSED_PAD src0_sel:WORD_0\n\t" \
	"v_cvt_f32_i32_sdwa v223, sext(%[g7]) dst_sel:DWORD dst_unused:UNUSED_PAD src0_sel:WORD_1\n\t" \
	"s_branch .Lput_end_%=\n\t" \
	".Lput_8_%=:\n\t" \
	"v_cvt_f32_i32_sdwa v224, sext(%[g0]) dst_sel:DWORD dst_unused:UNUSED_PAD src0_sel:WORD_0\n\t" \
	"v_cvt_f32_i32_sdwa v225, sext(%[g0]) dst_sel:DWORD dst_unused:UNUSED_PAD src0_sel:WORD_1\n\t" \
	"v_cvt_f32_i32_sdwa v226, sext(%[g1]) dst_sel:DWORD dst_unused:UNUSED_PAD src0_sel:WORD_0\n\t" \
	"v_cvt_f32_i32_sdwa v227, sext(%[g1]) dst_sel:DWORD dst_unused:UNUSED_PAD src0_sel:WORD_1\n\t" \
	"v_cvt_f32_i32_sdwa v228, sext(%[g2]) dst_sel:DWORD dst_unused:UNUSED_PAD src0_sel:WORD_0\n\t" \
	"v_cvt_f32_i32_sdwa v229, sext(%[g2]) dst_sel:DWORD dst_unused:UNUSED_PAD src0_sel:WORD_1\n\t" \
	"v_cvt_f32_i32_sdwa v230, sext(%[g3]) dst_sel:DWORD dst_unused:UNUSED_PAD src0_sel:WORD_0\n\t" \
	"v_cvt_f32_i32_sdwa v231, sext(%[g3]) dst_sel:DWORD dst_unused:UNUSED_PAD src0_sel:WORD_1\n\t" \
	"v_cvt_f32_i32_sdwa v232, sext(%[g4]) dst_sel:DWORD dst_unused:UNUSED_PAD src0_sel:WORD_0\n\t" \
	"v_cvt_f32_i32_sdwa v233, sext(%[g4]) dst_sel:DWORD dst_unused:UNUSED_PAD src0_sel:WORD_1\n\t" \
	"v_cvt_f32_i32_sdwa v234, sext(%[g5]) dst_sel:DWORD dst_unused:UNUSED_PAD src0_sel:WORD_0\n\t" \
	"v_cvt_f32_i32_sdwa v235, sext(%[g5]) dst_sel:DWORD dst_unused:UNUSED_PAD src0_sel:WORD_1\n\t" \
	"v_cvt_f32_i32_sdwa v236, sext(%[g6]) dst_sel:DWORD dst_unused:UNUSED_PAD src0_sel:WORD_0\n\t" \
	"v_cvt_f32_i32_sdwa v237, sext(%[g6]) dst_sel:DWORD dst_unused:UNUSED_PAD src0_sel:WORD_1\n\t" \
	"v_cvt_f32_i32_sdwa v238, sext(%[g7]) dst_sel:DWORD dst_unused:UNUSED_PAD src0_sel:WORD_0\n\t" \
	"v_cvt_f32_i32_sdwa v239, sext(%[g7]) dst_sel:DWORD dst_unused:UNUSED_PAD src0_sel:WORD_1\n\t" \
	"s_branch .Lput_end_%=\n\t" \
	".Lput_9_%=:\n\t" \
	"v_cvt_f32_i32_sdwa v240, sext(%[g0]) dst_sel:DWORD dst_unused:UNUSED_PAD src0_sel:WORD_0\n\t" \
	"v_cvt_f32_i32_sdwa v241, sext(%[g0]) dst_sel:DWORD dst_unused:UNUSED_PAD src0_sel:WORD_1\n\t" \
	"v_cvt_f32_i32_sdwa v242, sext(%[g1]) dst_sel:DWORD dst_unused:UNUSED_PAD src0_sel:WORD_0\n\t" \
	"v_cvt_f32_i32_sdwa v243, sext(%[g1]) dst_sel:DWORD dst_unused:UNUSED_PAD src0_sel:WORD_1\n\t" \
	"v_cvt_f32_i32_sdwa v244, sext(%[g2]) dst_sel:DWORD dst_unused:UNUSED_PAD src0_sel:WORD_0\n\t" \
	"v_cvt_f32_i32_sdwa v245, sext(%[g2]) dst_sel:DWORD dst_unused:UNUSED_PAD src0_sel:WORD_1\n\t" \
	"v_cvt_f32_i32_sdwa v246, sext(%[g3]) dst_sel:DWORD dst_unused:UNUSED_PAD src0_sel:WORD_0\n\t" \
	"v_cvt_f32_i32_sdwa v247, sext(%[g3]) dst_sel:DWORD dst_unused:UNUSED_PAD src0_sel:WORD_1\n\t" \
	"v_cvt_f32_i32_sdwa v248, sext(%[g4]) dst_sel:DWORD dst_unused:UNUSED_PAD src0_sel:WORD_0\n\t" \
	"v_cvt_f32_i32_sdwa v249, sext(%[g4]) dst_sel:DWORD dst_unused:UNUSED_PAD src0_sel:WORD_1\n\t" \
	"v_cvt_f32_i32_sdwa v250, sext(%[g5]) dst_sel:DWORD dst_unused:UNUSED_PAD src0_sel:WORD_0\n\t" \
	"v_cvt_f32_i32_sdwa v251, sext(%[g5]) dst_sel:DWORD dst_unused:UNUSED_PAD src0_sel:WORD_1\n\t" \
	"v_cvt_f32_i32_sdwa v252, sext(%[g6]) dst_sel:DWORD dst_unused:UNUSED_PAD src0_sel:WORD_0\n\t" \
	"v_cvt_f32_i32_sdwa v253, sext(%[g6]) dst_sel:DWORD dst_unused:UNUSED_PAD src0_sel:WORD_1\n\t" \
	"v_cvt_f32_i32_sdwa v254, sext(%[g7]) dst_sel:DWORD dst_unused:UNUSED_PAD src0_sel:WORD_0\n\t" \
	"v_cvt_f32_i32_sdwa v255, sext(%[g7]) dst_sel:DWORD dst_unused:UNUSED_PAD src0_sel:WORD_1\n\t" \
	"s_branch .Lput_end_%=\n\t" \
	".Lput_end_%=:\n\t" \
	"s_add_i32 %[base], %[base], 8\n\t" \
	"s_add_i32 %[rot], %[rot], 1\n\t" \
	"s_cmp_eq_u32 %[rot], 10\n\t" \
	"s_cselect_b32 %[rot], 0, %[rot]\n\t"
#define ROTWIN_PUT_U8_ASM \
	"s_nop 1\n\t" \
	"s_getpc_b64 vcc\n\t" \
	".Lput_pc_%=:\n\t" \
	"s_mul_i32 %[tmp], %[rot], (.Lput_1_%= - .Lput_0_%=)\n\t" \
	"s_add_u32 %[tmp], %[tmp], (.Lput_0_%= - .Lput_pc_%=)\n\t" \
	"s_add_u32 vcc_lo, vcc_lo, %[tmp]\n\t" \
	"s_addc_u32 vcc_hi, vcc_hi, 0\n\t" \
	"s_setpc_b64 vcc\n\t" \
	".Lput_0_%=:\n\t" \
	"v_cvt_f32_i32_sdwa v96, sext(%[g0]) dst_sel:DWORD dst_unused:UNUSED_PAD src0_sel:BYTE_0\n\t" \
	"v_cvt_f32_i32_sdwa v97, sext(%[g0]) dst_sel:DWORD dst_unused:UNUSED_PAD src0_sel:BYTE_1\n\t" \
	"v_cvt_f32_i32_sdwa v98, sext(%[g0]) dst_sel:DWORD dst_unused:UNUSED_PAD src0_sel:BYTE_2\n\t" \
	"v_cvt_f32_i32_sdwa v99, sext(%[g0]) dst_sel:DWORD dst_unused:UNUSED_PAD src0_sel:BYTE_3\n\t" \
	"v_cvt_f32_i32_sdwa v100, sext(%[g1]) dst_sel:DWORD dst_unused:UNUSED_PAD src0_sel:BYTE_0\n\t" \
	"v_cvt_f32_i32_sdwa v101, sext(%[g1]) dst_sel:DWORD dst_unused:UNUSED_PAD src0_sel:BYTE_1\n\t" \
	"v_cvt_f32_i32_sdwa v102, sext(%[g1]) dst_sel:DWORD dst_unused:UNUSED_PAD src0_sel:BYTE_2\n\t" \
	"v_cvt_f32_i32_sdwa v103, sext(%[g1]) dst_sel:DWORD dst_unused:UNUSED_PAD src0_sel:BYTE_3\n\t" \
	"v_cvt_f32_i32_sdwa v104, sext(%[g2]) dst_sel:DWORD dst_unused:UNUSED_PAD src0_sel:BYTE_0\n\t" \
	"v_cvt_f32_i32_sdwa v105, sext(%[g2]) dst_sel:DWORD dst_unused:UNUSED_PAD src0_sel:BYTE_1\n\t" \
	"v_cvt_f32_i32_sdwa v106, sext(%[g2]) dst_sel:DWORD dst_unused:UNUSED_PAD src0_sel:BYTE_2\n\t" \
	"v_cvt_f32_i32_sdwa v107, sext(%[g2]) dst_sel:DWORD dst_unused:UNUSED_PAD src0_sel:BYTE_3\n\t" \
	"v_cvt_f32_i32_sdwa v108, sext(%[g3]) dst_sel:DWORD dst_unused:UNUSED_PAD src0_sel:BYTE_0\n\t" \
	"v_cvt_f32_i32_sdwa v109, sext(%[g3]) dst_sel:DWORD dst_unused:UNUSED_PAD src0_sel:BYTE_1\n\t" \
	"v_cvt_f32_i32_sdwa v110, sext(%[g3]) dst_sel:DWORD dst_unused:UNUSED_PAD src0_sel:BYTE_2\n\t" \
	"v_cvt_f32_i32_sdwa v111, sext(%[g3]) dst_sel:DWORD dst_unused:UNUSED_PAD src0_sel:BYTE_3\n\t" \
	"s_branch .Lput_end_%=\n\t" \
	".Lput_1_%=:\n\t" \
	"v_cvt_f32_i32_sdwa v112, sext(%[g0]) dst_sel:DWORD dst_unused:UNUSED_PAD src0_sel:BYTE_0\n\t" \
	"v_cvt_f32_i32_sdwa v113, sext(%[g0]) dst_sel:DWORD dst_unused:UNUSED_PAD src0_sel:BYTE_1\n\t" \
	"v_cvt_f32_i32_sdwa v114, sext(%[g0]) dst_sel:DWORD dst_unused:UNUSED_PAD src0_sel:BYTE_2\n\t" \
	"v_cvt_f32_i32_sdwa v115, sext(%[g0]) dst_sel:DWORD dst_unused:UNUSED_PAD src0_sel:BYTE_3\n\t" \
	"v_cvt_f32_i32_sdwa v116, sext(%[g1]) dst_sel:DWORD dst_unused:UNUSED_PAD src0_sel:BYTE_0\n\t" \
	"v_cvt_f32_i32_sdwa v117, sext(%[g1]) dst_sel:DWORD dst_unused:UNUSED_PAD src0_sel:BYTE_1\n\t" \
	"v_cvt_f32_i32_sdwa v118, sext(%[g1]) dst_sel:DWORD dst_unused:UNUSED_PAD src0_sel:BYTE_2\n\t" \
	"v_cvt_f32_i32_sdwa v119, sext(%[g1]) dst_sel:DWORD dst_unused:UNUSED_PAD src0_sel:BYTE_3\n\t" \
	"v_cvt_f32_i32_sdwa v120, sext(%[g2]) dst_sel:DWORD dst_unused:UNUSED_PAD src0_sel:BYTE_0\n\t" \
	"v_cvt_f32_i32_sdwa v121, sext(%[g2]) dst_sel:DWORD dst_unused:UNUSED_PAD src0_sel:BYTE_1\n\t" \
	"v_cvt_f32_i32_sdwa v122, sext(%[g2]) dst_sel:DWORD dst_unused:UNUSED_PAD src0_sel:BYTE_2\n\t" \
	"v_cvt_f32_i32_sdwa v123, sext(%[g2]) dst_sel:DWORD dst_unused:UNUSED_PAD src0_sel:BYTE_3\n\t" \
	"v_cvt_f32_i32_sdwa v124, sext(%[g3]) dst_sel:DWORD dst_unused:UNUSED_PAD src0_sel:BYTE_0\n\t" \
	"v_cvt_f32_i32_sdwa v125, sext(%[g3]) dst_sel:DWORD dst_unused:UNUSED_PAD src0_sel:BYTE_1\n\t" \
	"v_cvt_f32_i32_sdwa v126, sext(%[g3]) dst_sel:DWORD dst_unused:UNUSED_PAD src0_sel:BYTE_2\n\t" \
	"v_cvt_f32_i32_sdwa v127, sext(%[g3]) dst_sel:DWORD dst_unused:UNUSED_PAD src0_sel:BYTE_3\n\t" \
	"s_branch .Lput_end_%=\n\t" \
	".Lput_2_%=:\n\t" \
	"v_cvt_f32_i32_sdwa v128, sext(%[g0]) dst_sel:DWORD dst_unused:UNUSED_PAD src0_sel:BYTE_0\n\t" \
	"v_cvt_f32_i32_sdwa v129, sext(%[g0]) dst_sel:DWORD dst_unused:UNUSED_PAD src0_sel:BYTE_1\n\t" \
	"v_cvt_f32_i32_sdwa v130, sext(%[g0]) dst_sel:DWORD dst_unused:UNUSED_PAD src0_sel:BYTE_2\n\t" \
	"v_cvt_f32_i32_sdwa v131, sext(%[g0]) dst_sel:DWORD dst_unused:UNUSED_PAD src0_sel:BYTE_3\n\t" \
	"v_cvt_f32_i32_sdwa v132, sext(%[g1]) dst_sel:DWORD dst_unused:UNUSED_PAD src0_sel:BYTE_0\n\t" \
	"v_cvt_f32_i32_sdwa v133, sext(%[g1]) dst_sel:DWORD dst_unused:UNUSED_PAD src0_sel:BYTE_1\n\t" \
	"v_cvt_f32_i32_sdwa v134, sext(%[g1]) dst_sel:DWORD dst_unused:UNUSED_PAD src0_sel:BYTE_2\n\t" \
	"v_cvt_f32_i32_sdwa v135, sext(%[g1]) dst_sel:DWORD dst_unused:UNUSED_PAD src0_sel:BYTE_3\n\t" \
	"v_cvt_f32_i32_sdwa v136, sext(%[g2]) dst_sel:DWORD dst_unused:UNUSED_PAD src0_sel:BYTE_0\n\t" \
	"v_cvt_f32_i32_sdwa v137, sext(%[g2]) dst_sel:DWORD dst_unused:UNUSED_PAD src0_sel:BYTE_1\n\t" \
	"v_cvt_f32_i32_sdwa v138, sext(%[g2]) dst_sel:DWORD dst_unused:UNUSED_PAD src0_sel:BYTE_2\n\t" \
	"v_cvt_f32_i32_sdwa v139, sext(%[g2]) dst_sel:DWORD dst_unused:UNUSED_PAD src0_sel:BYTE_3\n\t" \
	"v_cvt_f32_i32_sdwa v140, sext(%[g3]) dst_sel:DWORD dst_unused:UNUSED_PAD src0_sel:BYTE_0\n\t" \
	"v_cvt_f32_i32_sdwa v141, sext(%[g3]) dst_sel:DWORD dst_unused:UNUSED_PAD src0_sel:BYTE_1\n\t" \
	"v_cvt_f32_i32_sdwa v142, sext(%[g3]) dst_sel:DWORD dst_unused:UNUSED_PAD src0_sel:BYTE_2\n\t" \
	"v_cvt_f32_i32_sdwa v143, sext(%[g3]) dst_sel:DWORD dst_unused:UNUSED_PAD src0_sel:BYTE_3\n\t" \
	"s_branch .Lput_end_%=\n\t" \
	".Lput_3_%=:\n\t" \
	"v_cvt_f32_i32_sdwa v144, sext(%[g0]) dst_sel:DWORD dst_unused:UNUSED_PAD src0_sel:BYTE_0\n\t" \
	"v_cvt_f32_i32_sdwa v145, sext(%[g0]) dst_sel:DWORD dst_unused:UNUSED_PAD src0_sel:BYTE_1\n\t" \
	"v_cvt_f32_i32_sdwa v146, sext(%[g0]) dst_sel:DWORD dst_unused:UNUSED_PAD src0_sel:BYTE_2\n\t" \
	"v_cvt_f32_i32_sdwa v147, sext(%[g0]) dst_sel:DWORD dst_unused:UNUSED_PAD src0_sel:BYTE_3\n\t" \
	"v_cvt_f32_i32_sdwa v148, sext(%[g1]) dst_sel:DWORD dst_unused:UNUSED_PAD src0_sel:BYTE_0\n\t" \
	"v_cvt_f32_i32_sdwa v149, sext(%[g1]) dst_sel:DWORD dst_unused:UNUSED_PAD src0_sel:BYTE_1\n\t" \
	"v_cvt_f32_i32_sdwa v150, sext(%[g1]) dst_sel:DWORD dst_unused:UNUSED_PAD src0_sel:BYTE_2\n\t" \
	"v_cvt_f32_i32_sdwa v151, sext(%[g1]) dst_sel:DWORD dst_unused:UNUSED_PAD src0_sel:BYTE_3\n\t" \
	"v_cvt_f32_i32_sdwa v152, sext(%[g2]) dst_sel:DWORD dst_unused:UNUSED_PAD src0_sel:BYTE_0\n\t" \
	"v_cvt_f32_i32_sdwa v153, sext(%[g2]) dst_sel:DWORD dst_unused:UNUSED_PAD src0_sel:BYTE_1\n\t" \
	"v_cvt_f32_i32_sdwa v154, sext(%[g2]) dst_sel:DWORD dst_unused:UNUSED_PAD src0_sel:BYTE_2\n\t" \
	"v_cvt_f32_i32_sdwa v155, sext(%[g2]) dst_sel:DWORD dst_unused:UNUSED_PAD src0_sel:BYTE_3\n\t" \
	"v_cvt_f32_i32_sdwa v156, sext(%[g3]) dst_sel:DWORD dst_unused:UNUSED_PAD src0_sel:BYTE_0\n\t" \
	"v_cvt_f32_i32_sdwa v157, sext(%[g3]) dst_sel:DWORD dst_unused:UNUSED_PAD src0_sel:BYTE_1\n\t" \
	"v_cvt_f32_i32_sdwa v158, sext(%[g3]) dst_sel:DWORD dst_unused:UNUSED_PAD src0_sel:BYTE_2\n\t" \
	"v_cvt_f32_i32_sdwa v159, sext(%[g3]) dst_sel:DWORD dst_unused:UNUSED_PAD src0_sel:BYTE_3\n\t" \
// ... 28 lines not shown
	"v_cvt_f32_i32_sdwa v184, sext(%[g2]) dst_sel:DWORD dst_unused:UNUSED_PAD src0_sel:BYTE_0\n\t" \
	"v_cvt_f32_i32_sdwa v185, sext(%[g2]) dst_sel:DWORD dst_unused:UNUSED_PAD src0_sel:BYTE_1\n\t" \
	"v_cvt_f32_i32_sdwa v186, sext(%[g2]) dst_sel:DWORD dst_unused:UNUSED_PAD src0_sel:BYTE_2\n\t" \
	"v_cvt_f32_i32_sdwa v187, sext(%[g2]) dst_sel:DWORD dst_unused:UNUSED_PAD src0_sel:BYTE_3\n\t" \
	"v_cvt_f32_i32_sdwa v188, sext(%[g3]) dst_sel:DWORD dst_unused:UNUSED_PAD src0_sel:BYTE_0\n\t" \
	"v_cvt_f32_i32_sdwa v189, sext(%[g3]) dst_sel:DWORD dst_unused:UNUSED_PAD src0_sel:BYTE_1\n\t" \
	"v_cvt_f32_i32_sdwa v190, sext(%[g3]) dst_sel:DWORD dst_unused:UNUSED_PAD src0_sel:BYTE_2\n\t" \
	"v_cvt_f32_i32_sdwa v191, sext(%[g3]) dst_sel:DWORD dst_unused:UNUSED_PAD src0_sel:BYTE_3\n\t" \
	"s_branch .Lput_end_%=\n\t" \
	".Lput_6_%=:\n\t" \
	"v_cvt_f32_i32_sdwa v192, sext(%[g0]) dst_sel:DWORD dst_unused:UNUSED_PAD src0_sel:BYTE_0\n\t" \
	"v_cvt_f32_i32_sdwa v193, sext(%[g0]) dst_sel:DWORD dst_unused:UNUSED_PAD src0_sel:BYTE_1\n\t" \
	"v_cvt_f32_i32_sdwa v194, sext(%[g0]) dst_sel:DWORD dst_unused:UNUSED_PAD src0_sel:BYTE_2\n\t" \
	"v_cvt_f32_i32_sdwa v195, sext(%[g0]) dst_sel:DWORD dst_unused:UNUSED_PAD src0_sel:BYTE_3\n\t" \
	"v_cvt_f32_i32_sdwa v196, sext(%[g1]) dst_sel:DWORD dst_unused:UNUSED_PAD src0_sel:BYTE_0\n\t" \
	"v_cvt_f32_i32_sdwa v197, sext(%[g1]) dst_sel:DWORD dst_unused:UNUSED_PAD src0_sel:BYTE_1\n\t" \
	"v_cvt_f32_i32_sdwa v198, sext(%[g1]) dst_sel:DWORD dst_unused:UNUSED_PAD src0_sel:BYTE_2\n\t" \
	"v_cvt_f32_i32_sdwa v199, sext(%[g1]) dst_sel:DWORD dst_unused:UNUSED_PAD src0_sel:BYTE_3\n\t" \
	"v_cvt_f32_i32_sdwa v200, sext(%[g2]) dst_sel:DWORD dst_unused:UNUSED_PAD src0_sel:BYTE_0\n\t" \
	"v_cvt_f32_i32_sdwa v201, sext(%[g2]) dst_sel:DWORD dst_unused:UNUSED_PAD src0_sel:BYTE_1\n\t" \
	"v_cvt_f32_i32_sdwa v202, sext(%[g2]) dst_sel:DWORD dst_unused:UNUSED_PAD src0_sel:BYTE_2\n\t" \
	"v_cvt_f32_i32_sdwa v203, sext(%[g2]) dst_sel:DWORD dst_unused:UNUSED_PAD src0_sel:BYTE_3\n\t" \
	"v_cvt_f32_i32_sdwa v204, sext(%[g3]) dst_sel:DWORD dst_unused:UNUSED_PAD src0_sel:BYTE_0\n\t" \
	"v_cvt_f32_i32_sdwa v205, sext(%[g3]) dst_sel:DWORD dst_unused:UNUSED_PAD src0_sel:BYTE_1\n\t" \
	"v_cvt_f32_i32_sdwa v206, sext(%[g3]) dst_sel:DWORD dst_unused:UNUSED_PAD src0_sel:BYTE_2\n\t" \
	"v_cvt_f32_i32_sdwa v207, sext(%[g3]) dst_sel:DWORD dst_unused:UNUSED_PAD src0_sel:BYTE_3\n\t" \
	"s_branch .Lput_end_%=\n\t" \
	".Lput_7_%=:\n\t" \
	"v_cvt_f32_i32_sdwa v208, sext(%[g0]) dst_sel:DWORD dst_unused:UNUSED_PAD src0_sel:BYTE_0\n\t" \
	"v_cvt_f32_i32_sdwa v209, sext(%[g0]) dst_sel:DWORD dst_unused:UNUSED_PAD src0_sel:BYTE_1\n\t" \
	"v_cvt_f32_i32_sdwa v210, sext(%[g0]) dst_sel:DWORD dst_unused:UNUSED_PAD src0_sel:BYTE_2\n\t" \
	"v_cvt_f32_i32_sdwa v211, sext(%[g0]) dst_sel:DWORD dst_unused:UNUSED_PAD src0_sel:BYTE_3\n\t" \
	"v_cvt_f32_i32_sdwa v212, sext(%[g1]) dst_sel:DWORD dst_unused:UNUSED_PAD src0_sel:BYTE_0\n\t" \
	"v_cvt_f32_i32_sdwa v213, sext(%[g1]) dst_sel:DWORD dst_unused:UNUSED_PAD src0_sel:BYTE_1\n\t" \
	"v_cvt_f32_i32_sdwa v214, sext(%[g1]) dst_sel:DWORD dst_unused:UNUSED_PAD src0_sel:BYTE_2\n\t" \
	"v_cvt_f32_i32_sdwa v215, sext(%[g1]) dst_sel:DWORD dst_unused:UNUSED_PAD src0_sel:BYTE_3\n\t" \
	"v_cvt_f32_i32_sdwa v216, sext(%[g2]) dst_sel:DWORD dst_unused:UNUSED_PAD src0_sel:BYTE_0\n\t" \
	"v_cvt_f32_i32_sdwa v217, sext(%[g2]) dst_sel:DWORD dst_unused:UNUSED_PAD src0_sel:BYTE_1\n\t" \
	"v_cvt_f32_i32_sdwa v218, sext(%[g2]) dst_sel:DWORD dst_unused:UNUSED_PAD src0_sel:BYTE_2\n\t" \
	"v_cvt_f32_i32_sdwa v219, sext(%[g2]) dst_sel:DWORD dst_unused:UNUSED_PAD src0_sel:BYTE_3\n\t" \
	"v_cvt_f32_i32_sdwa v220, sext(%[g3]) dst_sel:DWORD dst_unused:UNUSED_PAD src0_sel:BYTE_0\n\t" \
	"v_cvt_f32_i32_sdwa v221, sext(%[g3]) dst_sel:DWORD dst_unused:UNUSED_PAD src0_sel:BYTE_1\n\t" \
	"v_cvt_f32_i32_sdwa v222, sext(%[g3]) dst_sel:DWORD dst_unused:UNUSED_PAD src0_sel:BYTE_2\n\t" \
	"v_cvt_f32_i32_sdwa v223, sext(%[g3]) dst_sel:DWORD dst_unused:UNUSED_PAD src0_sel:BYTE_3\n\t" \
	"s_branch .Lput_end_%=\n\t" \
	".Lput_8_%=:\n\t" \
	"v_cvt_f32_i32_sdwa v224, sext(%[g0]) dst_sel:DWORD dst_unused:UNUSED_PAD src0_sel:BYTE_0\n\t" \
	"v_cvt_f32_i32_sdwa v225, sext(%[g0]) dst_sel:DWORD dst_unused:UNUSED_PAD src0_sel:BYTE_1\n\t" \
	"v_cvt_f32_i32_sdwa v226, sext(%[g0]) dst_sel:DWORD dst_unused:UNUSED_PAD src0_sel:BYTE_2\n\t" \
	"v_cvt_f32_i32_sdwa v227, sext(%[g0]) dst_sel:DWORD dst_unused:UNUSED_PAD src0_sel:BYTE_3\n\t" \
	"v_cvt_f32_i32_sdwa v228, sext(%[g1]) dst_sel:DWORD dst_unused:UNUSED_PAD src0_sel:BYTE_0\n\t" \
	"v_cvt_f32_i32_sdwa v229, sext(%[g1]) dst_sel:DWORD dst_unused:UNUSED_PAD src0_sel:BYTE_1\n\t" \
	"v_cvt_f32_i32_sdwa v230, sext(%[g1]) dst_sel:DWORD dst_unused:UNUSED_PAD src0_sel:BYTE_2\n\t" \
	"v_cvt_f32_i32_sdwa v231, sext(%[g1]) dst_sel:DWORD dst_unused:UNUSED_PAD src0_sel:BYTE_3\n\t" \
	"v_cvt_f32_i32_sdwa v232, sext(%[g2]) dst_sel:DWORD dst_unused:UNUSED_PAD src0_sel:BYTE_0\n\t" \
	"v_cvt_f32_i32_sdwa v233, sext(%[g2]) dst_sel:DWORD dst_unused:UNUSED_PAD src0_sel:BYTE_1\n\t" \
	"v_cvt_f32_i32_sdwa v234, sext(%[g2]) dst_sel:DWORD dst_unused:UNUSED_PAD src0_sel:BYTE_2\n\t" \
	"v_cvt_f32_i32_sdwa v235, sext(%[g2]) dst_sel:DWORD dst_unused:UNUSED_PAD src0_sel:BYTE_3\n\t" \
	"v_cvt_f32_i32_sdwa v236, sext(%[g3]) dst_sel:DWORD dst_unused:UNUSED_PAD src0_sel:BYTE_0\n\t" \
	"v_cvt_f32_i32_sdwa v237, sext(%[g3]) dst_sel:DWORD dst_unused:UNUSED_PAD src0_sel:BYTE_1\n\t" \
	"v_cvt_f32_i32_sdwa v238, sext(%[g3]) dst_sel:DWORD dst_unused:UNUSED_PAD src0_sel:BYTE_2\n\t" \
	"v_cvt_f32_i32_sdwa v239, sext(%[g3]) dst_sel:DWORD dst_unused:UNUSED_PAD src0_sel:BYTE_3\n\t" \
	"s_branch .Lput_end_%=\n\t" \
	".Lput_9_%=:\n\t" \
	"v_cvt_f32_i32_sdwa v240, sext(%[g0]) dst_sel:DWORD dst_unused:UNUSED_PAD src0_sel:BYTE_0\n\t" \
	"v_cvt_f32_i32_sdwa v241, sext(%[g0]) dst_sel:DWORD dst_unused:UNUSED_PAD src0_sel:BYTE_1\n\t" \
	"v_cvt_f32_i32_sdwa v242, sext(%[g0]) dst_sel:DWORD dst_unused:UNUSED_PAD src0_sel:BYTE_2\n\t" \
	"v_cvt_f32_i32_sdwa v243, sext(%[g0]) dst_sel:DWORD dst_unused:UNUSED_PAD src0_sel:BYTE_3\n\t" \
	"v_cvt_f32_i32_sdwa v244, sext(%[g1]) dst_sel:DWORD dst_unused:UNUSED_PAD src0_sel:BYTE_0\n\t" \
	"v_cvt_f32_i32_sdwa v245, sext(%[g1]) dst_sel:DWORD dst_unused:UNUSED_PAD src0_sel:BYTE_1\n\t" \
	"v_cvt_f32_i32_sdwa v246, sext(%[g1]) dst_sel:DWORD dst_unused:UNUSED_PAD src0_sel:BYTE_2\n\t" \
	"v_cvt_f32_i32_sdwa v247, sext(%[g1]) dst_sel:DWORD dst_unused:UNUSED_PAD src0_sel:BYTE_3\n\t" \
	"v_cvt_f32_i32_sdwa v248, sext(%[g2]) dst_sel:DWORD dst_unused:UNUSED_PAD src0_sel:BYTE_0\n\t" \
	"v_cvt_f32_i32_sdwa v249, sext(%[g2]) dst_sel:DWORD dst_unused:UNUSED_PAD src0_sel:BYTE_1\n\t" \
	"v_cvt_f32_i32_sdwa v250, sext(%[g2]) dst_sel:DWORD dst_unused:UNUSED_PAD src0_sel:BYTE_2\n\t" \
	"v_cvt_f32_i32_sdwa v251, sext(%[g2]) dst_sel:DWORD dst_unused:UNUSED_PAD src0_sel:BYTE_3\n\t" \
	"v_cvt_f32_i32_sdwa v252, sext(%[g3]) dst_sel:DWORD dst_unused:UNUSED_PAD src0_sel:BYTE_0\n\t" \
	"v_cvt_f32_i32_sdwa v253, sext(%[g3]) dst_sel:DWORD dst_unused:UNUSED_PAD src0_sel:BYTE_1\n\t" \
	"v_cvt_f32_i32_sdwa v254, sext(%[g3]) dst_sel:DWORD dst_unused:UNUSED_PAD src0_sel:BYTE_2\n\t" \
	"v_cvt_f32_i32_sdwa v255, sext(%[g3]) dst_sel:DWORD dst_unused:UNUSED_PAD src0_sel:BYTE_3\n\t" \
	"s_branch .Lput_end_%=\n\t" \
	".Lput_end_%=:\n\t" \
	"s_add_i32 %[base], %[base], 8\n\t" \
	"s_add_i32 %[rot], %[rot], 1\n\t" \
	"s_cmp_eq_u32 %[rot], 10\n\t" \
	"s_cselect_b32 %[rot], 0, %[rot]\n\t"
#define ROTWIN_PUT_F32_ASM \
	"s_getpc_b64 vcc\n\t" \
	".Lput_pc_%=:\n\t" \
	"s_mul_i32 %[tmp], %[rot], (.Lput_1_%= - .Lput_0_%=)\n\t" \
	"s_add_u32 %[tmp], %[tmp], (.Lput_0_%= - .Lput_pc_%=)\n\t" \
	"s_add_u32 vcc_lo, vcc_lo, %[tmp]\n\t" \
	"s_addc_u32 vcc_hi, vcc_hi, 0\n\t" \
	"s_setpc_b64 vcc\n\t" \
	".Lput_0_%=:\n\t" \
	"v_mov_b32 v96, %[f0]\n\t" \
	"v_mov_b32 v97, %[f1]\n\t" \
	"v_mov_b32 v98, %[f2]\n\t" \
	"v_mov_b32 v99, %[f3]\n\t" \
	"v_mov_b32 v100, %[f4]\n\t" \
	"v_mov_b32 v101, %[f5]\n\t" \
	"v_mov_b32 v102, %[f6]\n\t" \
	"v_mov_b32 v103, %[f7]\n\t" \
	"v_mov_b32 v104, %[f8]\n\t" \
	"v_mov_b32 v105, %[f9]\n\t" \
	"v_mov_b32 v106, %[f10]\n\t" \
	"v_mov_b32 v107, %[f11]\n\t" \
	"v_mov_b32 v108, %[f12]\n\t" \
	"v_mov_b32 v109, %[f13]\n\t" \
	"v_mov_b32 v110, %[f14]\n\t" \
	"v_mov_b32 v111, %[f15]\n\t" \
	"s_branch .Lput_end_%=\n\t" \
	".Lput_1_%=:\n\t" \
	"v_mov_b32 v112, %[f0]\n\t" \
	"v_mov_b32 v113, %[f1]\n\t" \
	"v_mov_b32 v114, %[f2]\n\t" \
	"v_mov_b32 v115, %[f3]\n\t" \
	"v_mov_b32 v116, %[f4]\n\t" \
	"v_mov_b32 v117, %[f5]\n\t" \
	"v_mov_b32 v118, %[f6]\n\t" \
	"v_mov_b32 v119, %[f7]\n\t" \
	"v_mov_b32 v120, %[f8]\n\t" \
	"v_mov_b32 v121, %[f9]\n\t" \
	"v_mov_b32 v122, %[f10]\n\t" \
	"v_mov_b32 v123, %[f11]\n\t" \
	"v_mov_b32 v124, %[f12]\n\t" \
	"v_mov_b32 v125, %[f13]\n\t" \
	"v_mov_b32 v126, %[f14]\n\t" \
	"v_mov_b32 v127, %[f15]\n\t" \
	"s_branch .Lput_end_%=\n\t" \
	".Lput_2_%=:\n\t" \
	"v_mov_b32 v128, %[f0]\n\t" \
	"v_mov_b32 v129, %[f1]\n\t" \
	"v_mov_b32 v130, %[f2]\n\t" \
	"v_mov_b32 v131, %[f3]\n\t" \
	"v_mov_b32 v132, %[f4]\n\t" \
	"v_mov_b32 v133, %[f5]\n\t" \
	"v_mov_b32 v134, %[f6]\n\t" \
	"v_mov_b32 v135, %[f7]\n\t" \
	"v_mov_b32 v136, %[f8]\n\t" \
	"v_mov_b32 v137, %[f9]\n\t" \
	"v_mov_b32 v138, %[f10]\n\t" \
	"v_mov_b32 v139, %[f11]\n\t" \
	"v_mov_b32 v140, %[f12]\n\t" \
	"v_mov_b32 v141, %[f13]\n\t" \
	"v_mov_b32 v142, %[f14]\n\t" \
	"v_mov_b32 v143, %[f15]\n\t" \
	"s_branch .Lput_end_%=\n\t" \
	".Lput_3_%=:\n\t" \
	"v_mov_b32 v144, %[f0]\n\t" \
	"v_mov_b32 v145, %[f1]\n\t" \
	"v_mov_b32 v146, %[f2]\n\t" \
	"v_mov_b32 v147, %[f3]\n\t" \
	"v_mov_b32 v148, %[f4]\n\t" \
	"v_mov_b32 v149, %[f5]\n\t" \
	"v_mov_b32 v150, %[f6]\n\t" \
	"v_mov_b32 v151, %[f7]\n\t" \
	"v_mov_b32 v152, %[f8]\n\t" \
	"v_mov_b32 v153, %[f9]\n\t" \
	"v_mov_b32 v154, %[f10]\n\t" \
	"v_mov_b32 v155, %[f11]\n\t" \
	"v_mov_b32 v156, %[f12]\n\t" \
	"v_mov_b32 v157, %[f13]\n\t" \
	"v_mov_b32 v158, %[f14]\n\t" \
	"v_mov_b32 v159, %[f15]\n\t" \
	"s_branch .Lput_end_%=\n\t" \
// ... 27 lines not shown
	"v_mov_b32 v184, %[f8]\n\t" \
	"v_mov_b32 v185, %[f9]\n\t" \
	"v_mov_b32 v186, %[f10]\n\t" \
	"v_mov_b32 v187, %[f11]\n\t" \
	"v_mov_b32 v188, %[f12]\n\t" \
	"v_mov_b32 v189, %[f13]\n\t" \
	"v_mov_b32 v190, %[f14]\n\t" \
	"v_mov_b32 v191, %[f15]\n\t" \
	"s_branch .Lput_end_%=\n\t" \
	".Lput_6_%=:\n\t" \
	"v_mov_b32 v192, %[f0]\n\t" \
	"v_mov_b32 v193, %[f1]\n\t" \
	"v_mov_b32 v194, %[f2]\n\t" \
	"v_mov_b32 v195, %[f3]\n\t" \
	"v_mov_b32 v196, %[f4]\n\t" \
	"v_mov_b32 v197, %[f5]\n\t" \
	"v_mov_b32 v198, %[f6]\n\t" \
	"v_mov_b32 v199, %[f7]\n\t" \
	"v_mov_b32 v200, %[f8]\n\t" \
	"v_mov_b32 v201, %[f9]\n\t" \
	"v_mov_b32 v202, %[f10]\n\t" \
	"v_mov_b32 v203, %[f11]\n\t" \
	"v_mov_b32 v204, %[f12]\n\t" \
	"v_mov_b32 v205, %[f13]\n\t" \
	"v_mov_b32 v206, %[f14]\n\t" \
	"v_mov_b32 v207, %[f15]\n\t" \
	"s_branch .Lput_end_%=\n\t" \
	".Lput_7_%=:\n\t" \
	"v_mov_b32 v208, %[f0]\n\t" \
	"v_mov_b32 v209, %[f1]\n\t" \
	"v_mov_b32 v210, %[f2]\n\t" \
	"v_mov_b32 v211, %[f3]\n\t" \
	"v_mov_b32 v212, %[f4]\n\t" \
	"v_mov_b32 v213, %[f5]\n\t" \
	"v_mov_b32 v214, %[f6]\n\t" \
	"v_mov_b32 v215, %[f7]\n\t" \
	"v_mov_b32 v216, %[f8]\n\t" \
	"v_mov_b32 v217, %[f9]\n\t" \
	"v_mov_b32 v218, %[f10]\n\t" \
	"v_mov_b32 v219, %[f11]\n\t" \
	"v_mov_b32 v220, %[f12]\n\t" \
	"v_mov_b32 v221, %[f13]\n\t" \
	"v_mov_b32 v222, %[f14]\n\t" \
	"v_mov_b32 v223, %[f15]\n\t" \
	"s_branch .Lput_end_%=\n\t" \
	".Lput_8_%=:\n\t" \
	"v_mov_b32 v224, %[f0]\n\t" \
	"v_mov_b32 v225, %[f1]\n\t" \
	"v_mov_b32 v226, %[f2]\n\t" \
	"v_mov_b32 v227, %[f3]\n\t" \
	"v_mov_b32 v228, %[f4]\n\t" \
	"v_mov_b32 v229, %[f5]\n\t" \
	"v_mov_b32 v230, %[f6]\n\t" \
	"v_mov_b32 v231, %[f7]\n\t" \
	"v_mov_b32 v232, %[f8]\n\t" \
	"v_mov_b32 v233, %[f9]\n\t" \
	"v_mov_b32 v234, %[f10]\n\t" \
	"v_mov_b32 v235, %[f11]\n\t" \
	"v_mov_b32 v236, %[f12]\n\t" \
	"v_mov_b32 v237, %[f13]\n\t" \
	"v_mov_b32 v238, %[f14]\n\t" \
	"v_mov_b32 v239, %[f15]\n\t" \
	"s_branch .Lput_end_%=\n\t" \
	".Lput_9_%=:\n\t" \
	"v_mov_b32 v240, %[f0]\n\t" \
	"v_mov_b32 v241, %[f1]\n\t" \
	"v_mov_b32 v242, %[f2]\n\t" \
	"v_mov_b32 v243, %[f3]\n\t" \
	"v_mov_b32 v244, %[f4]\n\t" \
	"v_mov_b32 v245, %[f5]\n\t" \
	"v_mov_b32 v246, %[f6]\n\t" \
	"v_mov_b32 v247, %[f7]\n\t" \
	"v_mov_b32 v248, %[f8]\n\t" \
	"v_mov_b32 v249, %[f9]\n\t" \
	"v_mov_b32 v250, %[f10]\n\t" \
	"v_mov_b32 v251, %[f11]\n\t" \
	"v_mov_b32 v252, %[f12]\n\t" \
	"v_mov_b32 v253, %[f13]\n\t" \
	"v_mov_b32 v254, %[f14]\n\t" \
	"v_mov_b32 v255, %[f15]\n\t" \
	"s_branch .Lput_end_%=\n\t" \
	".Lput_end_%=:\n\t" \
	"s_add_i32 %[base], %[base], 8\n\t" \
	"s_add_i32 %[rot], %[rot], 1\n\t" \
	"s_cmp_eq_u32 %[rot], 10\n\t" \
	"s_cselect_b32 %[rot], 0, %[rot]\n\t"
#define ROTWIN_FIR_ACC_ASM \
	"ds_read_b128 v[80:83], %[addr] offset:0\n\t" \
	"ds_read_b128 v[84:87], %[addr] offset:16\n\t" \
	"s_getpc_b64 vcc\n\t" \
	".Lfira_pc_%=:\n\t" \
	"s_mul_i32 %[tmp], %[rot], (.Lfira_1_%= - .Lfira_0_%=)\n\t" \
	"s_add_u32 %[tmp], %[tmp], (.Lfira_0_%= - .Lfira_pc_%=)\n\t" \
	"s_add_u32 vcc_lo, vcc_lo, %[tmp]\n\t" \
	"s_addc_u32 vcc_hi, vcc_hi, 0\n\t" \
	"s_setpc_b64 vcc\n\t" \
	".Lfira_0_%=:\n\t" \
	"ds_read_b128 v[88:91], %[addr] offset:32\n\t" \
	"s_waitcnt lgkmcnt(2)\n\t" \
	"v_accvgpr_read_b32 v92, a96\n\t" \
	"v_accvgpr_read_b32 v93, a97\n\t" \
	"v_accvgpr_read_b32 v94, a98\n\t" \
	"v_accvgpr_read_b32 v95, a99\n\t" \
	"v_pk_mul_f32 v[92:93], v[92:93], v[80:81] op_sel:[0,0] op_sel_hi:[1,0]\n\t" \
	"v_pk_mul_f32 v[94:95], v[94:95], v[80:81] op_sel:[0,1] op_sel_hi:[1,1]\n\t" \
	"v_pk_add_f32 %[acc], %[acc], v[92:93]\n\t" \
	"v_accvgpr_read_b32 v92, a100\n\t" \
	"v_accvgpr_read_b32 v93, a101\n\t" \
	"v_pk_add_f32 %[acc], %[acc], v[94:95]\n\t" \
	"v_accvgpr_read_b32 v94, a102\n\t" \
	"v_accvgpr_read_b32 v95, a103\n\t" \
	"v_pk_mul_f32 v[92:93], v[92:93], v[82:83] op_sel:[0,0] op_sel_hi:[1,0]\n\t" \
	"v_pk_mul_f32 v[94:95], v[94:95], v[82:83] op_sel:[0,1] op_sel_hi:[1,1]\n\t" \
	"v_pk_add_f32 %[acc], %[acc], v[92:93]\n\t" \
	"v_pk_add_f32 %[acc], %[acc], v[94:95]\n\t" \
	"ds_read_b128 v[80:83], %[addr] offset:48\n\t" \
	"s_waitcnt lgkmcnt(2)\n\t" \
	"v_accvgpr_read_b32 v92, a104\n\t" \
	"v_accvgpr_read_b32 v93, a105\n\t" \
	"v_accvgpr_read_b32 v94, a106\n\t" \
	"v_accvgpr_read_b32 v95, a107\n\t" \
	"v_pk_mul_f32 v[92:93], v[92:93], v[84:85] op_sel:[0,0] op_sel_hi:[1,0]\n\t" \
	"v_pk_mul_f32 v[94:95], v[94:95], v[84:85] op_sel:[0,1] op_sel_hi:[1,1]\n\t" \
	"v_pk_add_f32 %[acc], %[acc], v[92:93]\n\t" \
	"v_accvgpr_read_b32 v92, a108\n\t" \
	"v_accvgpr_read_b32 v93, a109\n\t" \
	"v_pk_add_f32 %[acc], %[acc], v[94:95]\n\t" \
	"v_accvgpr_read_b32 v94, a110\n\t" \
	"v_accvgpr_read_b32 v95, a111\n\t" \
	"v_pk_mul_f32 v[92:93], v[92:93], v[86:87] op_sel:[0,0] op_sel_hi:[1,0]\n\t" \
	"v_pk_mul_f32 v[94:95], v[94:95], v[86:87] op_sel:[0,1] op_sel_hi:[1,1]\n\t" \
	"v_pk_add_f32 %[acc], %[acc], v[92:93]\n\t" \
	"v_pk_add_f32 %[acc], %[acc], v[94:95]\n\t" \
	"ds_read_b128 v[84:87], %[addr] offset:64\n\t" \
	"s_waitcnt lgkmcnt(2)\n\t" \
	"v_accvgpr_read_b32 v92, a112\n\t" \
	"v_accvgpr_read_b32 v93, a113\n\t" \
	"v_accvgpr_read_b32 v94, a114\n\t" \
	"v_accvgpr_read_b32 v95, a115\n\t" \
	"v_pk_mul_f32 v[92:93], v[92:93], v[88:89] op_sel:[0,0] op_sel_hi:[1,0]\n\t" \
	"v_pk_mul_f32 v[94:95], v[94:95], v[88:89] op_sel:[0,1] op_sel_hi:[1,1]\n\t" \
	"v_pk_add_f32 %[acc], %[acc], v[92:93]\n\t" \
	"v_accvgpr_read_b32 v92, a116\n\t" \
	"v_accvgpr_read_b32 v93, a117\n\t" \
	"v_pk_add_f32 %[acc], %[acc], v[94:95]\n\t" \
	"v_accvgpr_read_b32 v94, a118\n\t" \
	"v_accvgpr_read_b32 v95, a119\n\t" \
	"v_pk_mul_f32 v[92:93], v[92:93], v[90:91] op_sel:[0,0] op_sel_hi:[1,0]\n\t" \
	"v_pk_mul_f32 v[94:95], v[94:95], v[90:91] op_sel:[0,1] op_sel_hi:[1,1]\n\t" \
	"v_pk_add_f32 %[acc], %[acc], v[92:93]\n\t" \
	"v_pk_add_f32 %[acc], %[acc], v[94:95]\n\t" \
	"ds_read_b128 v[88:91], %[addr] offset:80\n\t" \
	"s_waitcnt lgkmcnt(2)\n\t" \
	"v_accvgpr_read_b32 v92, a120\n\t" \
	"v_accvgpr_read_b32 v93, a121\n\t" \
	"v_accvgpr_read_b32 v94, a122\n\t" \
	"v_accvgpr_read_b32 v95, a123\n\t" \
	"v_pk_mul_f32 v[92:93], v[92:93], v[80:81] op_sel:[0,0] op_sel_hi:[1,0]\n\t" \
	"v_pk_mul_f32 v[94:95], v[94:95], v[80:81] op_sel:[0,1] op_sel_hi:[1,1]\n\t" \
	"v_pk_add_f32 %[acc], %[acc], v[92:93]\n\t" \
	"v_accvgpr_read_b32 v92, a124\n\t" \
	"v_accvgpr_read_b32 v93, a125\n\t" \
	"v_pk_add_f32 %[acc], %[acc], v[94:95]\n\t" \
	"v_accvgpr_read_b32 v94, a126\n\t" \
	"v_accvgpr_read_b32 v95, a127\n\t" \
	"v_pk_mul_f32 v[92:93], v[92:93], v[82:83] op_sel:[0,0] op_sel_hi:[1,0]\n\t" \
// ... 6088 lines not shown
```

meteor_demod_amd/csrc/rotwin_body.h:

```cpp
#ifndef MDEMOD_ROTWIN_BODY_H
#define MDEMOD_ROTWIN_BODY_H

#include <hip/hip_runtime.h>
#include <stdint.h>

#include "demod_internal.h"
#include "demod_device.h"
#include "clock_jump.h"

#pragma clang fp contract(off)

#ifndef ROT_OQ_SYNC
#define ROT_OQ_SYNC 1
#endif
typedef float rot_sinlut_t;

namespace {

template <int FMT> struct RFmt;
template <> struct RFmt<16> { typedef uint32_t sample_t; enum { GDW = 4 }; };
template <> struct RFmt<8>  { typedef uint16_t sample_t; enum { GDW = 2 }; };
template <> struct RFmt<32> { typedef float2   sample_t; enum { GDW = 8 }; };

template <int FMT> struct RGran { uint32_t w[RFmt<FMT>::GDW]; };

template <int FMT>
__device__ __forceinline__ RGran<FMT>
rot_fetch(const typename RFmt<FMT>::sample_t *src, int m0, int n)
{
	typedef typename RFmt<FMT>::sample_t sample_t;
	RGran<FMT> g;
	if (m0 + 3 < n) {
		__builtin_memcpy(&g, src + m0, sizeof(g));
	} else {
		sample_t s[4];
#pragma unroll
		for (int u = 0; u < 4; u++) {
			if (m0 + u < n) s[u] = src[m0 + u];
			else __builtin_memset(&s[u], 0, sizeof(s[u]));
		}
		__builtin_memcpy(&g, s, sizeof(g));
	}
	return g;
}

__device__ __forceinline__ uint32_t
rot_mad24(uint32_t a, uint32_t b, uint32_t c)
{
	uint32_t r;
	asm("v_mad_u32_u24 %0, %1, %2, %3" : "=v"(r) : "v"(a), "s"(b), "v"(c));
	return r;
}

template <int K>
__device__ __forceinline__ float
blind_steps(float p, float f)
{
#pragma unroll
	for (int k = 0; k < K; k++) p = p + f;
	return p;
}

typedef int rot_i4 __attribute__((ext_vector_type(4)));
typedef const __attribute__((address_space(3))) rot_i4 *rot_clktab_t;
struct RotClockConsts { int k_safe, steps_need, interp; float f_hi; uint32_t magic; float inv; const cj_sched *jump; rot_clktab_t tab; };
template <int KS>
__device__ __forceinline__ void
rot_clock_fast(const RotClockConsts &K, float thr, int v_end, int v_fast_end, float &t_phase, float t_freq, int &isub, int &v_cur, int &bank, bool &fired, int jidx = -1)
{
	int k_safe = KS ? KS : K.k_safe;
	const int interp = K.interp;
	const bool jump = KS == 0 && jidx >= 0 && K.jump[jidx < 0 ? 0 : jidx].nb > 0;
	const cj_sched &J = K.jump[jidx < 0 ? 0 : jidx];
	const bool fast = (KS == 109 ? (t_phase > CJ109_P_LO && t_phase < CJ109_P_HI)
	                   : jump    ? (t_phase > J.floor && t_phase < J.hi)
	                             : (t_phase < thr - (float)k_safe * K.f_hi - 1e-3f))
	                  && (jump ? (v_cur + J.need < v_end) : (v_cur < v_fast_end));
	if (fast) {
		float p = t_phase;
		if (KS == 109) k_safe = clock_jump_109(p, t_freq, thr, K.inv);
		else if (KS) p = blind_steps<KS>(p, t_freq);
		else if (jump) k_safe = clock_jump_run(p, t_freq, thr, K.f_hi, K.inv, J);
		else {
			int k = k_safe;
			for (; k >= 16; k -= 16) p = blind_steps<16>(p, t_freq);
			if (k & 8) p = blind_steps<8>(p, t_freq);
			if (k & 4) p = blind_steps<4>(p, t_freq);
			if (k & 2) p = blind_steps<2>(p, t_freq);
			if (k & 1) p = p + t_freq;
		}
		const float p1 = p + t_freq, p2 = p1 + t_freq, p3 = p2 + t_freq, p4 = p3 + t_freq;
		const bool c1 = p1 >= thr, c2 = p2 >= thr, c3 = p3 >= thr, c4 = p4 >= thr;
		float ph = c3 ? p3 : p4;
		ph = c2 ? p2 : ph;
		ph = c1 ? p1 : ph;
		t_phase = ph;
		if ((KS == 14 || KS == 6) || (KS == 0 && K.tab)) {
			const uint32_t off = ((uint32_t)isub << 6) + (c1 ? 0u : 16u) + (c2 ? 0u : 16u) + (c3 ? 0u : 16u);
			const rot_i4 e = *reinterpret_cast<rot_clktab_t>(reinterpret_cast<const __attribute__((address_space(3))) unsigned char *>(K.tab) + off);
			v_cur += e.x;
			isub = e.z;
			bank = e.w;
		} else {
			const uint32_t w = (uint32_t)(isub + k_safe + 1 + (c1 ? 0 : 1) + (c2 ? 0 : 1) + (c3 ? 0 : 1));
			const uint32_t q = (interp == 1) ? w : __umulhi(w, K.magic);
			const int isub_new = (int)(w - q * (uint32_t)interp);
			v_cur += (int)q + (isub_new > 0 ? 1 : 0) - (isub > 0 ? 1 : 0);
			const int fire_sub = (isub_new == 0) ? interp - 1 : isub_new - 1;
			bank = interp - 1 - fire_sub;
			isub = isub_new;
		}
		fired = c4;
	}
}


template <class W, int FMT, int OQPSK, int KS, int LUT = 0>
__device__ __forceinline__ void
rotwin_demod(const DemodLaunch &L)
{
	typedef typename RFmt<FMT>::sample_t sample_t;
	constexpr int kBack = W::kBack, SLIDE = W::SLIDE, AMAX = W::AMAX, BLOCK = W::BLOCK, NCH = W::NW / W::SLIDE, GPS = W::SLIDE / 4;
	constexpr int NST = GPS * W::DEPTH;
	static_assert(W::DEPTH >= W::MAXSL, "a loop iteration may slide MAXSL times");
	constexpr int ROTN = W::ROTN, RING = W::RING, RGR = RING / 8;
	constexpr bool GATHER = W::GATHER;
	static_assert(RING == 32 || RING == 16, "output ring");
	constexpr int RS = W::REGSLOTS;
#ifndef ROT_PRIO
#define ROT_PRIO 1
#endif
#ifndef ROT_PRIO_LEVEL
#define ROT_PRIO_LEVEL 2
#endif
	constexpr int PRIO = ROT_PRIO;

	extern __shared__ __attribute__((aligned(16))) unsigned char lds[];
	float *ctab = reinterpret_cast<float *>(lds);
	float *lut = ctab + L.ctab_floats;
	enum { S_GAIN, S_BIAS_RE, S_BIAS_IM, S_PHASE, S_FREQ, S_ERR, S_FLAGS, S_TPREV, S_INPHASE, S_EVCALL, S_FIRSTLOCK, S_LASTV, S_COUNT };
	static_assert(S_COUNT == MDEMOD_RW_STATE_SLOTS, "host LDS sizing");
	uint32_t sl_addr = (uint32_t)(uintptr_t)(__attribute__((address_space(3))) unsigned char *)lds
	                   + 4u * (L.ctab_floats + 32u + (threadIdx.x >> 6) * (uint32_t)(S_COUNT * 64) + (threadIdx.x & 63u));
	asm("" : "+v"(sl_addr));
	float *sl = (float *)(__attribute__((address_space(3))) float *)(uintptr_t)sl_addr;
	int *sli = reinterpret_cast<int *>(sl);
	uint4 *stage = reinterpret_cast<uint4 *>(lut + 32 + (BLOCK / 64) * (S_COUNT * 64)) + threadIdx.x;
	const uint32_t ctab_addr = (uint32_t)(uintptr_t)(__attribute__((address_space(3))) unsigned char *)lds;
	W win;
	rot_sinlut_t *sintab = reinterpret_cast<rot_sinlut_t *>(stage - threadIdx.x + BLOCK * RGR);
	if constexpr (LUT) md_sin_lut_fill(sintab, (int)threadIdx.x, BLOCK);
	win.setup(ctab_addr + (uint32_t)(reinterpret_cast<unsigned char *>(stage - threadIdx.x + BLOCK * RGR) - lds) + (LUT ? MDEMOD_SIN_LUT_BYTES : 0));
	rot_i4 *clktab = reinterpret_cast<rot_i4 *>(reinterpret_cast<unsigned char *>(stage - threadIdx.x + BLOCK * RGR) + (LUT ? MDEMOD_SIN_LUT_BYTES : 0));

	const DemodConsts &C = L.c;
	const uint32_t stream = blockIdx.x * blockDim.x + threadIdx.x;
	const bool valid = stream < L.n_streams;

	for (uint32_t i = threadIdx.x; i < L.ctab_floats; i += blockDim.x) ctab[i] = L.ctab[i];
	if (threadIdx.x < 32) lut[threadIdx.x] = L.tanh_lut[threadIdx.x];
	const bool has_clktab = KS != 109 && C.clock_tab != nullptr;
	if (has_clktab)
		for (int i = (int)threadIdx.x; i < 4 * C.interp; i += (int)blockDim.x) clktab[i] = reinterpret_cast<const rot_i4 *>(C.clock_tab)[i];

	int n = 0;
	const sample_t *src = nullptr;
	if (valid) {
		n = (int)(L.n_samples_arr ? L.n_samples_arr[stream] : L.n_samples);
		const uint64_t off = L.iq_offset ? L.iq_offset[stream] : (uint64_t)stream * L.iq_stride;
		src = reinterpret_cast<const sample_t *>(L.iq) + off;
	}
	const int v_end = kBack + n;
	const int interp = C.interp;

	float t_phase = 0.0f, t_freq = C.t_center;
	int dual_state = 1;
	float r_gain = 1.0f, r_bias_re = 0.0f, r_bias_im = 0.0f, r_phase = 0.0f, r_freq = 0.0f;
	float r_err = 1000.0f, r_tprev = 0.0f;
	int r_flags = 0, r_lastv = -1;
	auto ld_err = [&]() -> float { return (RS & 1) ? r_err : sl[S_ERR * 64]; };
	auto st_err = [&](float v) { if (RS & 1) r_err = v; else sl[S_ERR * 64] = v; };
	auto ld_tprev = [&]() -> float { return (RS & 2) ? r_tprev : sl[S_TPREV * 64]; };
	auto st_tprev = [&](float v) { if (RS & 2) r_tprev = v; else sl[S_TPREV * 64] = v; };
	auto ld_flags = [&]() -> int { return (RS & 4) ? r_flags : sli[S_FLAGS * 64]; };
	auto st_flags = [&](int v) { if (RS & 4) r_flags = v; else sli[S_FLAGS * 64] = v; };
	auto ld_lastv = [&]() -> int { return (RS & 8) ? r_lastv : sli[S_LASTV * 64]; };
	auto st_lastv = [&](int v) { if (RS & 8) r_lastv = v; else sli[S_LASTV * 64] = v; };
	{
		float err = 1000.0f, t_prev = 0.0f, inph = 0.0f;
		int fl = MDEMOD_FLAG_UPDOWN_POS | (1 << MDEMOD_FLAG_DUAL_SHIFT);
		if (valid) {
			r_gain = L.st.agc_gain[stream]; r_bias_re = L.st.agc_bias_re[stream]; r_bias_im = L.st.agc_bias_im[stream];
			r_phase = L.st.pll_phase[stream]; r_freq = L.st.pll_freq[stream]; err = L.st.pll_err[stream];
			fl = L.st.flags[stream];
			t_phase = L.st.t_phase[stream]; t_freq = L.st.t_freq[stream]; t_prev = L.st.t_prev[stream];
			inph = L.st.inphase[stream];
		}
		dual_state = (fl >> MDEMOD_FLAG_DUAL_SHIFT) & 3;
		st_err(err);
		st_flags(fl & 7);
		st_tprev(t_prev); sl[S_INPHASE * 64] = inph;
		sli[S_EVCALL * 64] = 0; sli[S_FIRSTLOCK * 64] = -1; st_lastv(-1);
	}

	const float2 *hist_in = reinterpret_cast<const float2 *>(L.st.hist) + (size_t)(valid ? stream : 0) * kBack;
	if constexpr (!GATHER) {
		const float2 *hist = hist_in;
#pragma unroll 1
		for (int c = 0; c < kBack / SLIDE; c++) win.put_history(hist + c * SLIDE, valid, __builtin_amdgcn_readfirstlane(c));
#pragma unroll 1
		for (int c = 0; c < NCH - kBack / SLIDE; c++) {
			RGran<FMT> g[GPS];
#pragma unroll
			for (int i = 0; i < GPS; i++) g[i] = rot_fetch<FMT>(src, SLIDE * c + 4 * i, n);
			win.put_init(g, __builtin_amdgcn_readfirstlane(kBack / SLIDE + c));
		}
	}
	int g_load = (W::NW - kBack) / 4;
	RGran<FMT> stg[GATHER ? 1 : NST];
	if constexpr (!GATHER) {
#pragma unroll
		for (int i = 0; i < NST; i++) stg[i] = rot_fetch<FMT>(src, 4 * (g_load + i), n);
		g_load += NST;
	}

	__syncthreads();

	int rot = 0;
	int slot = 1;
	int base = 0;
	if constexpr (W::SCALAR_SLIDE) asm("s_mov_b32 %0, 0\n\ts_mov_b32 %1, 0" : "=s"(rot), "=s"(base));
	int isub = 0, bank = interp - 1;
	bool fired = false;
	bool done = !valid || n == 0;
	constexpr int V_DONE = 0x3FFFFFFF;
	int v_cur = done ? V_DONE : kBack - 1;
	uint32_t sym_call = 0;
	RotClockConsts K;
	K.k_safe = C.step_safe; K.f_hi = C.step_fmax; K.magic = C.interp_magic; K.interp = C.interp; K.inv = C.step_inv;
	K.steps_need = ((KS == 109 ? CJ109_MAX_STEPS : C.step_safe) + 4 + C.interp - 1) / C.interp;
	K.jump = C.jump;
	K.tab = has_clktab ? (rot_clktab_t)clktab : (rot_clktab_t)0;
	const int v_fast_end = v_end - K.steps_need;
	float k_t_alpha = C.t_alpha, k_t_beta = C.t_beta, k_t_center = C.t_center, k_pll_alpha = C.pll_alpha, k_pll_beta = C.pll_beta;
	if constexpr (W::VCONST) asm("" : "+v"(k_t_alpha), "+v"(k_t_beta), "+v"(k_t_center), "+v"(k_pll_alpha), "+v"(k_pll_beta));

	int n_wave_max = n;
	for (int o = 32; o > 0; o >>= 1) {
		const int other = __shfl_xor(n_wave_max, o);
		n_wave_max = other > n_wave_max ? other : n_wave_max;
	}
	n_wave_max = __builtin_amdgcn_readfirstlane(n_wave_max);
	const uint64_t guard64 = 4ull * (uint64_t)(n_wave_max + kBack) * (uint64_t)interp + 4096ull;
	uint32_t guard = guard64 > 0xFFFFFFFFull ? 0xFFFFFFFFu : (uint32_t)guard64;
#ifdef ROT_EXP_TIMING
	uint64_t tacc[5] = { 0, 0, 0, 0, 0 }, tlast = clock64();
	uint32_t n_iter = 0, n_fir = 0, n_slide = 0, n_wslow = 0;
#define ROT_TICK(i) do { const uint64_t t_ = clock64(); tacc[i] += t_ - tlast; tlast = t_; } while (0)
#else
#define ROT_TICK(i) do { } while (0)
#endif
	do {
		ROT_TICK(4);
		if (!fired && !done) {
			const float thr = OQPSK ? (float)dual_state * MD_PI_F : MD_TWO_PI_F;
			rot_clock_fast<KS>(K, thr, v_end, v_fast_end, t_phase, t_freq, isub, v_cur, bank, fired);
			while (!fired && !done) {
				if (isub == 0) {
					if (v_cur + 1 >= v_end) { done = true; v_cur = V_DONE; break; }
					v_cur++;
				}
				t_phase = t_phase + t_freq;
				bank = interp - 1 - isub;
				isub = (isub + 1 == interp) ? 0 : isub + 1;
				if (t_phase >= thr) fired = true;
			}
		}
		if constexpr (GATHER) if (md_all(v_cur == V_DONE)) break;
		ROT_TICK(0);
#ifdef ROT_EXP_TIMING
		n_iter++;
#endif

		bool all_done = false;
		if constexpr (!GATHER)
#pragma unroll
		for (int r = 0; r < W::MAXSL; r++) {
			const int a_now = v_cur - kBack - base;
			if (md_all(a_now >= SLIDE)) {
				if (md_all(v_cur == V_DONE)) { all_done = true; break; }
				RGran<FMT> g[GPS];
#pragma unroll
				for (int i = 0; i < GPS; i++) g[i] = stg[i];
				if constexpr (W::SCALAR_SLIDE) win.slide(g, rot, base);
				else {
					win.put(g, __builtin_amdgcn_readfirstlane(rot));
					rot = __builtin_amdgcn_readfirstlane((rot == ROTN - 1) ? 0 : rot + 1);
					base = __builtin_amdgcn_readfirstlane(base + SLIDE);
				}
#pragma unroll
				for (int i = 0; i + GPS < NST; i++) stg[i] = stg[i + GPS];
				const int m_new = 4 * g_load;
				if (md_all(m_new + SLIDE - 1 < n)) {
#pragma unroll
					for (int i = 0; i < GPS; i++) __builtin_memcpy(&stg[NST - GPS + i], src + m_new + 4 * i, sizeof(RGran<FMT>));
				} else {
#pragma unroll
					for (int i = 0; i < GPS; i++) stg[NST - GPS + i] = rot_fetch<FMT>(src, m_new + 4 * i, n);
				}
				g_load += GPS;
			}
		}
		if (all_done) break;

		ROT_TICK(1);
		const int a = v_cur - kBack - base;
		if (fired && (GATHER || a <= AMAX) && (!(OQPSK && ROT_OQ_SYNC) || dual_state == slot)) {
			fired = false;
			cf32 y;
			if constexpr (GATHER) win.fir_gather(ctab_addr, src, hist_in, v_cur, n, bank, C, y.re, y.im);
			else win.fir(ctab_addr, a, bank, C, W::SCALAR_SLIDE ? rot : __builtin_amdgcn_readfirstlane(rot), y.re, y.im);
			if (PRIO) __builtin_amdgcn_s_setprio(ROT_PRIO_LEVEL);
			ROT_TICK(2);
#ifdef ROT_EXP_TIMING
			n_fir++;
#endif

			y = md_agc<(KS == 14 && !OQPSK && LUT)>(y, r_gain, r_bias_re, r_bias_im);
			uint32_t fl = (uint32_t)ld_flags();
			PllWord pll;
			pll.phase = r_phase; pll.freq = r_freq;
			pll.err = ld_err();

			float sn, cs;
			if constexpr (LUT) {
				sn = md_sin_from_code_lut(sintab, md_turn_code<false>(-pll.phase));
				cs = md_sin_from_code_lut(sintab, md_turn_code<false>((float)((double)(-pll.phase) + MD_HALF_PI_D)));
			} else {
				sn = md_fast_sin<false>(-pll.phase);
				cs = md_fast_cos<false>(-pll.phase);
			}
			bool emit = true;
			float out_re, out_im;
			if (OQPSK) {
				float inphase = sl[S_INPHASE * 64];
				const int rail = ROT_OQ_SYNC ? slot : dual_state;
				if (rail == 1) { inphase = y.re * cs - y.im * sn; emit = false; sl[S_INPHASE * 64] = inphase; }
				out_re = inphase;
				out_im = y.re * sn + y.im * cs;
				dual_state = 3 - rail;
			} else {
				out_re = y.re * cs - y.im * sn;
				out_im = y.re * sn + y.im * cs;
			}
			md_nco_advance<true>(pll.phase, pll.freq);

			if (emit) {
				const bool again = (v_cur == ld_lastv());
				st_lastv(v_cur);
				if (__builtin_expect(md_any(again), 0)) { if (again) sym_call--; }
				float t_prev = ld_tprev();
				md_timing_update(t_phase, t_freq, t_prev, k_t_alpha, k_t_beta, k_t_center, C.t_maxdev, out_im);
				st_tprev(t_prev);
			}
			rot_clock_fast<KS>(K, OQPSK ? (float)dual_state * MD_PI_F : MD_TWO_PI_F, v_end, v_fast_end, t_phase, t_freq, isub, v_cur, bank, fired,
			                   OQPSK ? (ROT_OQ_SYNC ? 2 - slot : -1) : 0);
#ifdef ROT_EXP_TIMING
			if (!fired) n_slide++;
			if (md_any(!fired)) n_wslow++;
#endif
			if (emit) {
				uint32_t first = 0;
				const uint32_t changed = md_pll_update_packed(pll, fl, lut, k_pll_alpha, k_pll_beta, C.pll_fmax, out_re, out_im, first);
				if (__builtin_expect(changed != 0, 0)) {
					if (first) sli[S_FIRSTLOCK * 64] = (int)sym_call;
					const int ev_call = sli[S_EVCALL * 64];
					if (ev_call < MDEMOD_MAX_LOCK_EVENTS) {
						mdemod_lock_event ev;
						ev.symbol = L.st.n_symbols[stream] + sym_call; ev.locked = (int)(fl & 1u); ev.pad = 0;
						L.st.events[(size_t)stream * MDEMOD_MAX_LOCK_EVENTS + ev_call] = ev;
					}
					sli[S_EVCALL * 64] = ev_call + 1;
				}
				const uint32_t sym = (uint32_t)(md_quantise(out_re) & 0xFF) | ((uint32_t)(md_quantise(out_im) & 0xFF) << 8);
				const uint32_t k = sym_call & (uint32_t)(RING - 1);
				reinterpret_cast<uint16_t *>(stage + (k >> 3) * BLOCK)[k & 7u] = (uint16_t)sym;
				sym_call++;
				if (__builtin_expect((sym_call & (uint32_t)(RING - 1)) == 0, 0)) {
					int8_t *soft_out = L.soft + (size_t)stream * L.soft_stride * 2;
					if (__builtin_expect(sym_call <= L.soft_cap, 1)) {
						int8_t *dst = soft_out + 2 * (size_t)(sym_call - RING);
#pragma unroll
						for (int g4 = 0; g4 < RGR; g4++) {
							const uint4 qv = stage[g4 * BLOCK];
							__builtin_memcpy(dst + 16 * g4, &qv, 16);
							asm volatile("" ::: "memory");
						}
					} else {
						fl |= 8;
						for (uint32_t i = 0; i < (uint32_t)RING && sym_call - RING + i < L.soft_cap; i++)
							*reinterpret_cast<uint16_t *>(soft_out + 2 * (size_t)(sym_call - RING + i)) =
							    reinterpret_cast<const uint16_t *>(stage + (i >> 3) * BLOCK)[i & 7u];
					}
				}
			}
			r_phase = pll.phase; r_freq = pll.freq;
			st_err(pll.err);
			st_flags((int)fl);
			if (PRIO == 1) __builtin_amdgcn_s_setprio(0);
			ROT_TICK(3);
		}
		if (OQPSK && ROT_OQ_SYNC) slot = __builtin_amdgcn_readfirstlane(3 - slot);
	} while (--guard);
#ifdef ROT_EXP_TIMING
	for (int o = 32; o > 0; o >>= 1) n_slide += __shfl_xor(n_slide, o);
	if (blockIdx.x == 100 && threadIdx.x == 0)
		printf("ROT_TIMING iters %u firs %u (lanes left to the stepping loop: %u of the wave's, in %u firings) cycles: clock %llu slide %llu fir %llu scalar %llu latch %llu\n", n_iter, n_fir, n_slide, n_wslow,
		       (unsigned long long)tacc[0], (unsigned long long)tacc[1], (unsigned long long)tacc[2], (unsigned long long)tacc[3], (unsigned long long)tacc[4]);
#endif

	if (guard == 0) st_flags(ld_flags() | 8);

	uint32_t stream_e = stream;
	asm volatile("" : "+v"(stream_e));
	int8_t *soft_e = L.soft + (size_t)stream_e * L.soft_stride * 2;
	int overflow = (ld_flags() >> 3) & 1;

	if (valid) {
		const uint32_t r = sym_call & (uint32_t)(RING - 1), sb = sym_call - r;
		for (uint32_t g = 0; g < (r >> 3); g++) {
			if (sb + 8 * g + 8 <= L.soft_cap) { const uint4 qv = stage[g * BLOCK]; __builtin_memcpy(soft_e + 2 * (size_t)(sb + 8 * g), &qv, 16); }
			else for (uint32_t i = 0; i < 8; i++) {
				if (sb + 8 * g + i < L.soft_cap) *reinterpret_cast<uint16_t *>(soft_e + 2 * (size_t)(sb + 8 * g + i)) = reinterpret_cast<const uint16_t *>(stage + g * BLOCK)[i];
				else overflow = 1;
			}
		}
		for (uint32_t i = r & ~7u; i < r; i++) {
			if (sb + i < L.soft_cap) *reinterpret_cast<uint16_t *>(soft_e + 2 * (size_t)(sb + i)) = reinterpret_cast<const uint16_t *>(stage + (i >> 3) * BLOCK)[i & 7u];
			else overflow = 1;
		}
	}

	if (valid) {
		const int fl = ld_flags();
		L.st.agc_gain[stream_e] = r_gain; L.st.agc_bias_re[stream_e] = r_bias_re; L.st.agc_bias_im[stream_e] = r_bias_im;
		L.st.pll_phase[stream_e] = r_phase; L.st.pll_freq[stream_e] = r_freq; L.st.pll_err[stream_e] = ld_err();
		L.st.flags[stream_e] = (fl & 7) | (dual_state << MDEMOD_FLAG_DUAL_SHIFT);
		L.st.t_phase[stream_e] = t_phase; L.st.t_freq[stream_e] = t_freq; L.st.t_prev[stream_e] = ld_tprev();
		L.st.inphase[stream_e] = sl[S_INPHASE * 64];
		const uint64_t nsym0 = L.st.n_symbols[stream_e];
		const int first_lock_call = sli[S_FIRSTLOCK * 64];
		L.st.n_samples[stream_e] += (uint64_t)n;
		L.st.n_symbols[stream_e] = nsym0 + sym_call;
		if (first_lock_call >= 0) L.st.first_lock[stream_e] = (int64_t)(nsym0 + (uint32_t)first_lock_call);
		L.st.sym_this_call[stream_e] = sym_call;
		L.st.ev_this_call[stream_e] = (uint32_t)sli[S_EVCALL * 64];
		L.st.overflow[stream_e] = overflow;

		float2 *hist = reinterpret_cast<float2 *>(L.st.hist) + (size_t)stream_e * kBack;
		for (int k = 0; k < kBack; k++) {
			const int idx = n + k;
			float2 h;
			if (idx < kBack) h = hist[idx];
			else {
				const sample_t raw = src[idx - kBack];
				if constexpr (FMT == 16) h = make_float2((float)(int)(int16_t)(raw & 0xFFFFu), (float)((int)raw >> 16));
				else if constexpr (FMT == 8) h = make_float2((float)((int)(raw & 0xFFu) - 128), (float)((int)(raw >> 8) - 128));
				else h = raw;
			}
			hist[k] = h;
		}
	}
}


}

#endif
```

Baseline: 274,300.

## Track slide and fire thresholds as scalar positions in the rot window loop

The scalar-slide window now keeps three scalar positions (window start, next slide threshold, fire limit), advanced inside the slide assembly. The per-iteration slide and fire tests become direct compares against these instead of recomputing offsets from base. The slide-path mask also enables a wave-uniform refill bound from the minimum n, an optional scalar-base global load path with per-lane 32-bit offsets, and a single-slide loop shape that leaves through the guard counter. This cuts per-iteration scalar and vector arithmetic and branching in the hot loop, at the cost of a few extra scalar registers and more template complexity; the default uses mask 1 for QPSK and 15 for OQPSK.

```diff
diff --git a/meteor_demod_amd/_capi.py b/meteor_demod_amd/_capi.py
--- a/meteor_demod_amd/_capi.py
+++ b/meteor_demod_amd/_capi.py
@@ -133,6 +133,7 @@
     "mdemod_clock_table": (C.c_int, [C.c_int32, C.c_int32, _P(C.c_int32), C.c_uint32]),
     "mdemod_plan_clock_table": (C.c_int, [C.c_void_p, _P(C.c_int32), C.c_uint32]),
     "mdemod_plan_launch": (C.c_int, [C.c_void_p, _P(C.c_int32)]),
+    "mdemod_rot_refill_reach": (C.c_uint64, []),
     "mdemod_device_count": (C.c_int, []),
     "mdemod_demodulate_recording_host": (C.c_int, [_P(MdemodParams), _P(MdemodRecordingOpts), C.c_void_p, C.c_uint64,
                                                    C.c_void_p, C.c_uint64, _P(MdemodRecordingReport)]),
diff --git a/meteor_demod_amd/csrc/demod_api.cpp b/meteor_demod_amd/csrc/demod_api.cpp
--- a/meteor_demod_amd/csrc/demod_api.cpp
+++ b/meteor_demod_amd/csrc/demod_api.cpp
@@ -10,6 +10,7 @@
 #include "demod_host.h"
 #include "demod_internal.h"
 #include "hip_host.h"
+#include "rot_slide_addr.h"
 
 struct mdemod_ctx {
 	mdemod_params params;
@@ -773,6 +774,12 @@
 	return rc;
 } MDEMOD_API_CATCH
 
+uint64_t
+mdemod_rot_refill_reach(void)
+{
+	return rot_saddr_max_dist();
+}
+
 int
 mdemod_plan_launch(const mdemod_params *params, int32_t out[MDEMOD_PLAN_LAUNCH_WORDS])
 try { MDEMOD_API_ENTER
diff --git a/meteor_demod_amd/csrc/demod_kernel_gat.hip b/meteor_demod_amd/csrc/demod_kernel_gat.hip
--- a/meteor_demod_amd/csrc/demod_kernel_gat.hip
+++ b/meteor_demod_amd/csrc/demod_kernel_gat.hip
@@ -28,7 +28,7 @@
 template <int KT, int FMT>
 struct WinG {
 	static constexpr int G = GFmt<FMT>::G, kTaps = KT, kBack = KT - 1, AMAX = G - 1, NS = KT + AMAX, NW = 4 * ((NS + 3) / 4), SLIDE = 4, MAXSL = 1, DEPTH = 1,
-	                     BLOCK = MDEMOD_RW_BLOCK, ROTN = 1, RING = 32, REGSLOTS = 0;
+	                     BLOCK = MDEMOD_RW_BLOCK, ROTN = 1, RING = 32, REGSLOTS = 0, SLIDE_PATH = 0;
 	static constexpr bool GATHER = true, SCALAR_SLIDE = false, VCONST = false;
 	static_assert(NS % G == 0 && NS / G <= 36, "whole 16-byte loads, and few enough of them to stay in registers");
 	typedef typename RFmt<FMT>::sample_t sample_t;
diff --git a/meteor_demod_amd/csrc/demod_kernel_rot.hip b/meteor_demod_amd/csrc/demod_kernel_rot.hip
--- a/meteor_demod_amd/csrc/demod_kernel_rot.hip
+++ b/meteor_demod_amd/csrc/demod_kernel_rot.hip
@@ -33,33 +33,33 @@
 #endif
 }
 
-template <int FMT> __device__ __forceinline__ void rot_put(const RGran<FMT> &a, const RGran<FMT> &b, int &q, int &base);
+template <int FMT> __device__ __forceinline__ void rot_put(const RGran<FMT> &a, const RGran<FMT> &b, int &q, int &base, int &ps, int &pf);
 template <> __device__ __forceinline__ void
-rot_put<16>(const RGran<16> &a, const RGran<16> &b, int &q, int &base)
+rot_put<16>(const RGran<16> &a, const RGran<16> &b, int &q, int &base, int &ps, int &pf)
 {
 	int tmp;
 	asm volatile(ROTWIN_PUT_S16_ASM
-	             : [tmp] "=&s"(tmp), [rot] "+s"(q), [base] "+s"(base)
+	             : [tmp] "=&s"(tmp), [rot] "+s"(q), [base] "+s"(base), [ps] "+s"(ps), [pf] "+s"(pf)
 	             : [g0] "v"(a.w[0]), [g1] "v"(a.w[1]), [g2] "v"(a.w[2]), [g3] "v"(a.w[3]),
 	               [g4] "v"(b.w[0]), [g5] "v"(b.w[1]), [g6] "v"(b.w[2]), [g7] "v"(b.w[3])
 	             : "vcc", "scc", "v255", "memory");
 }
 template <> __device__ __forceinline__ void
-rot_put<8>(const RGran<8> &a, const RGran<8> &b, int &q, int &base)
+rot_put<8>(const RGran<8> &a, const RGran<8> &b, int &q, int &base, int &ps, int &pf)
 {
 	const uint32_t g0 = a.w[0] ^ 0x80808080u, g1 = a.w[1] ^ 0x80808080u, g2 = b.w[0] ^ 0x80808080u, g3 = b.w[1] ^ 0x80808080u;
 	int tmp;
 	asm volatile(ROTWIN_PUT_U8_ASM
-	             : [tmp] "=&s"(tmp), [rot] "+s"(q), [base] "+s"(base)
+	             : [tmp] "=&s"(tmp), [rot] "+s"(q), [base] "+s"(base), [ps] "+s"(ps), [pf] "+s"(pf)
 	             : [g0] "v"(g0), [g1] "v"(g1), [g2] "v"(g2), [g3] "v"(g3)
 	             : "vcc", "scc", "v255", "memory");
 }
 __device__ __forceinline__ void
-rot_put_floats(const uint32_t (&f)[16], int &q, int &base)
+rot_put_floats(const uint32_t (&f)[16], int &q, int &base, int &ps, int &pf)
 {
 	int tmp;
 	asm volatile(ROTWIN_PUT_F32_ASM
-	             : [tmp] "=&s"(tmp), [rot] "+s"(q), [base] "+s"(base)
+	             : [tmp] "=&s"(tmp), [rot] "+s"(q), [base] "+s"(base), [ps] "+s"(ps), [pf] "+s"(pf)
 	             : [f0] "v"(f[0]), [f1] "v"(f[1]), [f2] "v"(f[2]), [f3] "v"(f[3]), [f4] "v"(f[4]), [f5] "v"(f[5]), [f6] "v"(f[6]), [f7] "v"(f[7]),
 	               [f8] "v"(f[8]), [f9] "v"(f[9]), [f10] "v"(f[10]), [f11] "v"(f[11]), [f12] "v"(f[12]), [f13] "v"(f[13]), [f14] "v"(f[14]), [f15] "v"(f[15])
 	             : "vcc", "scc", "v255", "memory");
@@ -67,23 +67,24 @@
 __device__ __forceinline__ void
 rot_put_floats(const uint32_t (&f)[16], int q)
 {
-	int base = 0;
-	rot_put_floats(f, q, base);
+	int base = 0, ps = 0, pf = 0;
+	rot_put_floats(f, q, base, ps, pf);
 }
 template <> __device__ __forceinline__ void
-rot_put<32>(const RGran<32> &a, const RGran<32> &b, int &q, int &base)
+rot_put<32>(const RGran<32> &a, const RGran<32> &b, int &q, int &base, int &ps, int &pf)
 {
 	uint32_t f[16];
 #pragma unroll
 	for (int i = 0; i < 8; i++) { f[i] = a.w[i]; f[8 + i] = b.w[i]; }
-	rot_put_floats(f, q, base);
-}
-
-template <int FMT, int COMPACT = 0, int BLK = MDEMOD_RW_BLOCK, int VC = 0, int RSL = 0>
+	rot_put_floats(f, q, base, ps, pf);
+}
+
+template <int FMT, int COMPACT = 0, int BLK = MDEMOD_RW_BLOCK, int VC = 0, int RSL = 0, int SLP = 0>
 struct WinF {
 	static constexpr int kTaps = 65, kBack = 64, NW = 80, SLIDE = 8, AMAX = NW - kTaps, MAXSL = 1, DEPTH = 1, BLOCK = BLK, ROTN = NW / SLIDE, RING = 32;
 	static constexpr bool GATHER = false;
 	static constexpr bool SCALAR_SLIDE = true;
+	static constexpr int SLIDE_PATH = SLP;
 	static constexpr bool VCONST = VC != 0;
 	static_assert(SLIDE == ROTWIN_SLIDE && ROTN == ROTWIN_NCH, "the slide's assembly counts for itself");
 	__device__ __forceinline__ void setup(uint32_t) {}
@@ -100,9 +101,9 @@
 		}
 		rot_put_floats(f, q);
 	}
-	__device__ static __forceinline__ void put(const RGran<FMT> (&g)[2], int q) { int base = 0; rot_put<FMT>(g[0], g[1], q, base); }
+	__device__ static __forceinline__ void put(const RGran<FMT> (&g)[2], int q) { int base = 0, ps = 0, pf = 0; rot_put<FMT>(g[0], g[1], q, base, ps, pf); }
 	__device__ static __forceinline__ void put_init(const RGran<FMT> (&g)[2], int q) { put(g, q); }
-	__device__ static __forceinline__ void slide(const RGran<FMT> (&g)[2], int &rot, int &base) { rot_put<FMT>(g[0], g[1], rot, base); }
+	__device__ static __forceinline__ void slide(const RGran<FMT> (&g)[2], int &rot, int &pos0, int &pos_slide, int &pos_fire) { rot_put<FMT>(g[0], g[1], rot, pos0, pos_slide, pos_fire); }
 	__device__ static __forceinline__ void fir(uint32_t ctab_addr, int a, int bank, const DemodConsts &C, int rot, float &re, float &im)
 	{
 		const int o = AMAX - a;
@@ -179,7 +180,7 @@
 template <int BLK, int NA, int MSL>
 struct WinH {
 	static constexpr int NR = 10, SLIDE = 8, NW = SLIDE * (NR + NA), kTaps = NA == 10 ? 129 : 65, kBack = kTaps - 1, AMAX = NW - kTaps, MAXSL = MSL, DEPTH = MSL,
-	                     BLOCK = BLK, ROTN = NR, RING = 32, REGSLOTS = 0;
+	                     BLOCK = BLK, ROTN = NR, RING = 32, REGSLOTS = 0, SLIDE_PATH = 0;
 	static constexpr bool GATHER = false, SCALAR_SLIDE = false, VCONST = false;
 	static_assert((NA == 10 || NA == 2 || NA == 5) && AMAX == (NA == 5 ? 55 : 31) && kBack % SLIDE == 0, "wide (160 slots, 129 taps), mid (96 slots, 65 taps) or far (120 slots, 65 taps)");
 	__device__ __forceinline__ void setup(uint32_t) {}
@@ -246,11 +247,17 @@
 #endif
 template <int FMT, int OQPSK, int KS, int COMPACT, int LUT>
 constexpr int rot_regslots() { return 15; }
+#ifndef ROT_SLIDE_PATH
+#define ROT_SLIDE_PATH -1
+#endif
+template <int FMT, int OQPSK, int KS, int COMPACT, int LUT>
+constexpr int rot_slide_path() { return ROT_SLIDE_PATH >= 0 ? ROT_SLIDE_PATH : (OQPSK ? 15 : 1); }
 template <int FMT, int OQPSK, int KS, int COMPACT, int LUT>
 __global__ void __launch_bounds__(LUT ? MDEMOD_RW_LUT_BLOCK : MDEMOD_RW_BLOCK, 2) __attribute__((amdgpu_num_vgpr(ROTWIN_LIMIT / 2)))
 demod_kernel_rot(const DemodLaunch L)
 {
-	rotwin_demod<WinF<FMT, COMPACT, LUT ? MDEMOD_RW_LUT_BLOCK : MDEMOD_RW_BLOCK, ROT_VCONST, rot_regslots<FMT, OQPSK, KS, COMPACT, LUT>()>, FMT, OQPSK, KS, LUT>(L);
+	rotwin_demod<WinF<FMT, COMPACT, LUT ? MDEMOD_RW_LUT_BLOCK : MDEMOD_RW_BLOCK, ROT_VCONST, rot_regslots<FMT, OQPSK, KS, COMPACT, LUT>(),
+	                  rot_slide_path<FMT, OQPSK, KS, COMPACT, LUT>()>, FMT, OQPSK, KS, LUT>(L);
 }
 
 template <int FMT, int OQPSK, int KS, int COMPACT = 0, int LUT = 0>
diff --git a/meteor_demod_amd/csrc/demod_kernel_rotp.hip b/meteor_demod_amd/csrc/demod_kernel_rotp.hip
--- a/meteor_demod_amd/csrc/demod_kernel_rotp.hip
+++ b/meteor_demod_amd/csrc/demod_kernel_rotp.hip
@@ -79,7 +79,7 @@
 template <int GEO, int FMT>
 struct WinP {
 	static constexpr int kTaps = GeoP<GEO>::kTaps, kBack = kTaps - 1, NW = GeoP<GEO>::NW, SLIDE = 16, AMAX = NW - kTaps,
-	                     MAXSL = GeoP<GEO>::MAXSL, DEPTH = GeoP<GEO>::DEPTH, BLOCK = GeoP<GEO>::BLOCK, NCH = NW / SLIDE, GD = FMT == 16 ? 16 : 8, REGSLOTS = 0, ROTN = NCH, RING = 32;
+	                     MAXSL = GeoP<GEO>::MAXSL, DEPTH = GeoP<GEO>::DEPTH, BLOCK = GeoP<GEO>::BLOCK, NCH = NW / SLIDE, GD = FMT == 16 ? 16 : 8, REGSLOTS = 0, SLIDE_PATH = 0, ROTN = NCH, RING = 32;
 	static constexpr bool GATHER = false, SCALAR_SLIDE = false, VCONST = false;
 	__device__ __forceinline__ void setup(uint32_t) {}
 	static_assert(kBack % SLIDE == 0 && NW % SLIDE == 0, "history and window are whole chunks");
diff --git a/meteor_demod_amd/csrc/gen_rotwin_asm.py b/meteor_demod_amd/csrc/gen_rotwin_asm.py
--- a/meteor_demod_amd/csrc/gen_rotwin_asm.py
+++ b/meteor_demod_amd/csrc/gen_rotwin_asm.py
@@ -120,6 +120,8 @@
         L += ["s_branch .Lput_end_%="]
     L += [".Lput_end_%=:"]
     L += ["s_add_i32 %%[base], %%[base], %d" % SLIDE,
+          "s_add_i32 %%[ps], %%[ps], %d" % SLIDE,
+          "s_add_i32 %%[pf], %%[pf], %d" % SLIDE,
           "s_add_i32 %[rot], %[rot], 1",
           "s_cmp_eq_u32 %%[rot], %d" % NCH,
           "s_cselect_b32 %[rot], 0, %[rot]"]
diff --git a/meteor_demod_amd/csrc/mdemod_internal_api.h b/meteor_demod_amd/csrc/mdemod_internal_api.h
--- a/meteor_demod_amd/csrc/mdemod_internal_api.h
+++ b/meteor_demod_amd/csrc/mdemod_internal_api.h
@@ -43,6 +43,8 @@
 int  mdemod_clock_table(int32_t interp, int32_t k_safe, int32_t *out, uint32_t cap_entries);
 int  mdemod_plan_clock_table(const mdemod_params *params, int32_t *out, uint32_t cap_entries);
 
+uint64_t mdemod_rot_refill_reach(void);
+
 enum { MDEMOD_LAUNCH_LAT = 0, MDEMOD_LAUNCH_GAT = 1, MDEMOD_LAUNCH_ROTH = 2, MDEMOD_LAUNCH_ROT = 3, MDEMOD_LAUNCH_ROTP = 4, MDEMOD_LAUNCH_V1 = 5 };
 #define MDEMOD_PLAN_LAUNCH_WORDS 16
 int  mdemod_plan_launch(const mdemod_params *params, int32_t out[MDEMOD_PLAN_LAUNCH_WORDS]);
diff --git a/meteor_demod_amd/csrc/rot_slide_addr.h b/meteor_demod_amd/csrc/rot_slide_addr.h
--- /dev/null
+++ b/meteor_demod_amd/csrc/rot_slide_addr.h
@@ -0,0 +1,59 @@
+#ifndef MDEMOD_ROT_SLIDE_ADDR_H
+#define MDEMOD_ROT_SLIDE_ADDR_H
+
+#include <stdint.h>
+
+#if defined(__HIPCC__) || defined(__CUDACC__)
+#define ROT_SADDR_HD __host__ __device__
+#else
+#define ROT_SADDR_HD
+#endif
+
+#define ROT_SADDR_OFFSET_BITS 32
+
+ROT_SADDR_HD constexpr uint64_t
+rot_saddr_max_dist()
+{
+	return (1ull << ROT_SADDR_OFFSET_BITS) - 1ull;
+}
+
+ROT_SADDR_HD constexpr uint64_t
+rot_saddr_key(uint64_t addr, bool valid)
+{
+	return valid ? addr : ~0ull;
+}
+
+ROT_SADDR_HD constexpr bool
+rot_saddr_lane_ok(uint64_t addr, bool valid, uint64_t lo)
+{
+	return !valid || (addr >= lo && addr - lo <= rot_saddr_max_dist());
+}
+
+ROT_SADDR_HD constexpr uint32_t
+rot_saddr_dist(uint64_t addr, bool valid, uint64_t lo, bool wave_ok)
+{
+	return (valid && wave_ok) ? (uint32_t)(addr - lo) : 0u;
+}
+
+ROT_SADDR_HD constexpr int
+rot_refill_pos_end(int n_min, int slide, int m_pos)
+{
+	return n_min - (slide - 1) - m_pos;
+}
+
+struct RotSaddrWave { uint64_t lo; bool ok; };
+
+ROT_SADDR_HD constexpr RotSaddrWave
+rot_saddr_wave(const uint64_t (&addr)[64], uint64_t valid_mask)
+{
+	uint64_t lo = ~0ull;
+	for (int l = 0; l < 64; l++) {
+		const uint64_t k = rot_saddr_key(addr[l], (valid_mask >> l) & 1);
+		lo = k < lo ? k : lo;
+	}
+	bool ok = true;
+	for (int l = 0; l < 64; l++) ok = ok && rot_saddr_lane_ok(addr[l], (valid_mask >> l) & 1, lo);
+	return RotSaddrWave{ lo, ok };
+}
+
+#endif
diff --git a/meteor_demod_amd/csrc/rotwin_asm.h b/meteor_demod_amd/csrc/rotwin_asm.h
--- a/meteor_demod_amd/csrc/rotwin_asm.h
+++ b/meteor_demod_amd/csrc/rotwin_asm.h
@@ -2270,6 +2270,8 @@
 	"s_branch .Lput_end_%=\n\t" \
 	".Lput_end_%=:\n\t" \
 	"s_add_i32 %[base], %[base], 8\n\t" \
+	"s_add_i32 %[ps], %[ps], 8\n\t" \
+	"s_add_i32 %[pf], %[pf], 8\n\t" \
 	"s_add_i32 %[rot], %[rot], 1\n\t" \
 	"s_cmp_eq_u32 %[rot], 10\n\t" \
 	"s_cselect_b32 %[rot], 0, %[rot]\n\t"
@@ -2464,6 +2466,8 @@
 	"s_branch .Lput_end_%=\n\t" \
 	".Lput_end_%=:\n\t" \
 	"s_add_i32 %[base], %[base], 8\n\t" \
+	"s_add_i32 %[ps], %[ps], 8\n\t" \
+	"s_add_i32 %[pf], %[pf], 8\n\t" \
 	"s_add_i32 %[rot], %[rot], 1\n\t" \
 	"s_cmp_eq_u32 %[rot], 10\n\t" \
 	"s_cselect_b32 %[rot], 0, %[rot]\n\t"
@@ -2657,6 +2661,8 @@
 	"s_branch .Lput_end_%=\n\t" \
 	".Lput_end_%=:\n\t" \
 	"s_add_i32 %[base], %[base], 8\n\t" \
+	"s_add_i32 %[ps], %[ps], 8\n\t" \
+	"s_add_i32 %[pf], %[pf], 8\n\t" \
 	"s_add_i32 %[rot], %[rot], 1\n\t" \
 	"s_cmp_eq_u32 %[rot], 10\n\t" \
 	"s_cselect_b32 %[rot], 0, %[rot]\n\t"
diff --git a/meteor_demod_amd/csrc/rotwin_body.h b/meteor_demod_amd/csrc/rotwin_body.h
--- a/meteor_demod_amd/csrc/rotwin_body.h
+++ b/meteor_demod_amd/csrc/rotwin_body.h
@@ -7,6 +7,7 @@
 #include "demod_internal.h"
 #include "demod_device.h"
 #include "clock_jump.h"
+#include "rot_slide_addr.h"
 
 #pragma clang fp contract(off)
 
@@ -127,6 +128,9 @@
 	constexpr bool GATHER = W::GATHER;
 	static_assert(RING == 32 || RING == 16, "output ring");
 	constexpr int RS = W::REGSLOTS;
+	constexpr int SLP = W::SLIDE_PATH;
+	static_assert(SLP == 0 || (W::SCALAR_SLIDE && !GATHER && W::MAXSL == 1 && W::DEPTH == 1), "the scalar slide path is the std window's");
+	static_assert(!(SLP & 4) || (SLP & 2), "the scalar-base refill is chosen by the scalar bounds test");
 #ifndef ROT_PRIO
 #define ROT_PRIO 1
 #endif
@@ -217,6 +221,7 @@
 		}
 	}
 	int g_load = (W::NW - kBack) / 4;
+	constexpr int g_load_first = (W::NW - kBack) / 4 + NST;
 	RGran<FMT> stg[GATHER ? 1 : NST];
 	if constexpr (!GATHER) {
 #pragma unroll
@@ -229,7 +234,10 @@
 	int rot = 0;
 	int slot = 1;
 	int base = 0;
-	if constexpr (W::SCALAR_SLIDE) asm("s_mov_b32 %0, 0\n\ts_mov_b32 %1, 0" : "=s"(rot), "=s"(base));
+	int pos0 = kBack, pos_slide = kBack + SLIDE, pos_fire = kBack + AMAX + 1;
+	if constexpr (W::SCALAR_SLIDE)
+		asm("s_mov_b32 %0, 0\n\ts_mov_b32 %1, %4\n\ts_mov_b32 %2, %5\n\ts_mov_b32 %3, %6"
+		    : "=s"(rot), "=s"(pos0), "=s"(pos_slide), "=s"(pos_fire) : "n"(kBack), "n"(kBack + SLIDE), "n"(kBack + AMAX + 1));
 	int isub = 0, bank = interp - 1;
 	bool fired = false;
 	bool done = !valid || n == 0;
@@ -251,8 +259,36 @@
 		n_wave_max = other > n_wave_max ? other : n_wave_max;
 	}
 	n_wave_max = __builtin_amdgcn_readfirstlane(n_wave_max);
+	constexpr int M_POS = 4 * g_load_first - SLIDE - kBack;
+	int pos_whole_end = 0;
+	if constexpr (SLP & 2) {
+		int n_wave_min = n;
+		for (int o = 32; o > 0; o >>= 1) {
+			const int other = __shfl_xor(n_wave_min, o);
+			n_wave_min = other < n_wave_min ? other : n_wave_min;
+		}
+		pos_whole_end = rot_refill_pos_end(__builtin_amdgcn_readfirstlane(n_wave_min), SLIDE, M_POS);
+	}
+	typedef const __attribute__((address_space(1))) unsigned char *rot_gptr_t;
+	rot_gptr_t sptr = (rot_gptr_t)0;
+	uint32_t src_dist = 0;
+	int pos_saddr_end = 0;
+	if constexpr (SLP & 4) {
+		const uint64_t addr = (uint64_t)(uintptr_t)src;
+		uint64_t lo = rot_saddr_key(addr, valid);
+		for (int o = 32; o > 0; o >>= 1) {
+			const uint64_t other = __shfl_xor((unsigned long long)lo, o);
+			lo = other < lo ? other : lo;
+		}
+		lo = ((uint64_t)(uint32_t)__builtin_amdgcn_readfirstlane((int)(uint32_t)(lo >> 32)) << 32) | (uint32_t)__builtin_amdgcn_readfirstlane((int)(uint32_t)lo);
+		const bool wave_ok = md_all(rot_saddr_lane_ok(addr, valid, lo));
+		src_dist = rot_saddr_dist(addr, valid, lo, wave_ok);
+		pos_saddr_end = wave_ok ? pos_whole_end : 0;
+		sptr = (rot_gptr_t)(uintptr_t)lo + (size_t)(4 * g_load_first) * sizeof(sample_t);
+	}
 	const uint64_t guard64 = 4ull * (uint64_t)(n_wave_max + kBack) * (uint64_t)interp + 4096ull;
 	uint32_t guard = guard64 > 0xFFFFFFFFull ? 0xFFFFFFFFu : (uint32_t)guard64;
+	bool finished = false;
 #ifdef ROT_EXP_TIMING
 	uint64_t tacc[5] = { 0, 0, 0, 0, 0 }, tlast = clock64();
 	uint32_t n_iter = 0, n_fir = 0, n_slide = 0, n_wslow = 0;
@@ -282,17 +318,15 @@
 		n_iter++;
 #endif
 
-		bool all_done = false;
-		if constexpr (!GATHER)
-#pragma unroll
-		for (int r = 0; r < W::MAXSL; r++) {
-			const int a_now = v_cur - kBack - base;
-			if (md_all(a_now >= SLIDE)) {
-				if (md_all(v_cur == V_DONE)) { all_done = true; break; }
+		auto slide_due = [&]() -> bool {
+			return (SLP & 1) ? md_all(v_cur >= pos_slide) : md_all((W::SCALAR_SLIDE ? v_cur - pos0 : v_cur - kBack - base) >= SLIDE);
+		};
+		auto slide_once = [&]() {
+			if constexpr (!GATHER) {
 				RGran<FMT> g[GPS];
 #pragma unroll
 				for (int i = 0; i < GPS; i++) g[i] = stg[i];
-				if constexpr (W::SCALAR_SLIDE) win.slide(g, rot, base);
+				if constexpr (W::SCALAR_SLIDE) win.slide(g, rot, pos0, pos_slide, pos_fire);
 				else {
 					win.put(g, __builtin_amdgcn_readfirstlane(rot));
 					rot = __builtin_amdgcn_readfirstlane((rot == ROTN - 1) ? 0 : rot + 1);
@@ -300,22 +334,49 @@
 				}
 #pragma unroll
 				for (int i = 0; i + GPS < NST; i++) stg[i] = stg[i + GPS];
-				const int m_new = 4 * g_load;
-				if (md_all(m_new + SLIDE - 1 < n)) {
-#pragma unroll
-					for (int i = 0; i < GPS; i++) __builtin_memcpy(&stg[NST - GPS + i], src + m_new + 4 * i, sizeof(RGran<FMT>));
-				} else {
-#pragma unroll
-					for (int i = 0; i < GPS; i++) stg[NST - GPS + i] = rot_fetch<FMT>(src, m_new + 4 * i, n);
+				auto refill_lanes = [&]() {
+					const int m_new = (SLP & 2) ? pos0 + M_POS : 4 * g_load;
+					if ((SLP & 2) ? pos0 < pos_whole_end : md_all(m_new + SLIDE - 1 < n)) {
+#pragma unroll
+						for (int i = 0; i < GPS; i++) __builtin_memcpy(&stg[NST - GPS + i], src + m_new + 4 * i, sizeof(RGran<FMT>));
+					} else {
+#pragma unroll
+						for (int i = 0; i < GPS; i++) stg[NST - GPS + i] = rot_fetch<FMT>(src, m_new + 4 * i, n);
+					}
+				};
+				if constexpr ((SLP & 4) != 0) {
+					if (__builtin_expect(pos0 < pos_saddr_end, 1)) {
+						asm volatile("" : "+v"(src_dist));
+#pragma unroll
+						for (int i = 0; i < GPS; i++) __builtin_memcpy(&stg[NST - GPS + i], sptr + (size_t)src_dist + i * sizeof(RGran<FMT>), sizeof(RGran<FMT>));
+					} else refill_lanes();
+					sptr += SLIDE * sizeof(sample_t);
+				} else refill_lanes();
+				g_load += GPS;
+			}
+		};
+		bool all_done = false;
+		if constexpr ((SLP & 8) != 0) {
+			if (slide_due()) {
+				if (md_all(v_cur == V_DONE)) { guard = 1; finished = true; }
+				else slide_once();
+			}
+		} else if constexpr (!GATHER) {
+#pragma unroll
+			for (int r = 0; r < W::MAXSL; r++) {
+				if (slide_due()) {
+					if (md_all(v_cur == V_DONE)) { all_done = true; break; }
+					slide_once();
 				}
-				g_load += GPS;
 			}
 		}
 		if (all_done) break;
 
 		ROT_TICK(1);
-		const int a = v_cur - kBack - base;
-		if (fired && (GATHER || a <= AMAX) && (!(OQPSK && ROT_OQ_SYNC) || dual_state == slot)) {
+		const bool inside = (SLP & 1) ? v_cur < pos_fire : (W::SCALAR_SLIDE ? v_cur - pos0 : v_cur - kBack - base) <= AMAX;
+		const bool fire_now = fired && (GATHER || inside) && (!(OQPSK && ROT_OQ_SYNC) || dual_state == slot);
+		if ((SLP & 8) ? __builtin_expect(fire_now, 1) : fire_now) {
+			const int a = W::SCALAR_SLIDE ? v_cur - pos0 : v_cur - kBack - base;
 			fired = false;
 			cf32 y;
 			if constexpr (GATHER) win.fir_gather(ctab_addr, src, hist_in, v_cur, n, bank, C, y.re, y.im);
@@ -419,7 +480,7 @@
 		       (unsigned long long)tacc[0], (unsigned long long)tacc[1], (unsigned long long)tacc[2], (unsigned long long)tacc[3], (unsigned long long)tacc[4]);
 #endif
 
-	if (guard == 0) st_flags(ld_flags() | 8);
+	if (guard == 0 && !finished) st_flags(ld_flags() | 8);
 
 	uint32_t stream_e = stream;
 	asm volatile("" : "+v"(stream_e));
```

New measurement: 275,000 (median of 6 runs). Within noise of the previous version (+0.3%).
